# uw-x/AcousticSwarms-Speech

Hardware: AMD Instinct MI355X
Metric: TDoA candidates/sec (shift+normalise+spot forward+energies) (higher is better)
Workload: dtype f32 via f16x3 split-operand MFMA (fp32 accumulate); 1 GPU; configs[2] scene: 5-speaker reverberant mixture (image sources), 7 mics, T=48000 samples (BASELINE's '3 s @ 16 kHz' sample count; the reference pipeline and this scene generator run at 48 kHz, where it is a 1 s clip -- the reference-native 3 s is extras.T144000), fine-stage (Strict=1) candidate batch of one mixture, FULL spot net 47.27 M params, seeded random weights; internal_batch=256, parallelism=candidate-shard x1

## Files before the change

### acousticswarms-speech_amd/csrc/asw_common.cpp

```cpp
#include "asw_common.h"

#include <cmath>
#include <cstdlib>

namespace asw {
char* err_buf() {
  static thread_local char buf[512] = {0};
  return buf;
}
int set_error(int code, const char* fmt, ...) {
  va_list ap;
  va_start(ap, fmt);
  vsnprintf(err_buf(), 512, fmt, ap);
  va_end(ap);
  return code;
}
int SmemAttr::ensure(const void* kern, size_t want) {
  int dev = 0;
  ASW_HIP(hipGetDevice(&dev));
  if (dev < 0 || dev >= kMaxDev) return set_error(ASW_ERR_ARG, "device ordinal %d out of range", dev);
  if (bytes[dev] >= want) return ASW_OK;
  ASW_HIP(hipFuncSetAttribute(kern, hipFuncAttributeMaxDynamicSharedMemorySize, (int)want));
  bytes[dev] = want;
  return ASW_OK;
}
}

extern "C" const char* asw_last_error(void) { return asw::err_buf(); }
extern "C" int asw_abi_version(void) { return 3; }

extern "C" int asw_split_weights_f16(const float* w, size_t n, uint16_t* hi, uint16_t* lo, int32_t* w_shift) {
  ASW_CHECK_ARG(w && hi && lo && w_shift, "split_weights: null pointer");
  float mx = 0.f;
  for (size_t i = 0; i < n; ++i) { const float a = w[i] < 0 ? -w[i] : w[i]; if (a > mx || a != a) mx = a; }
  ASW_CHECK_ARG(mx == mx && mx < 3.0e38f, "split_weights: non-finite weight");
  int shift = 0;
  if (mx > 0.f) {
    int e;
    (void)frexpf(mx, &e);
    shift = 11 - e;
    if (shift > 24) shift = 24;
    if (shift < -24) shift = -24;
  }
  const float sc = ldexpf(1.0f, shift);
  for (size_t i = 0; i < n; ++i) {
    float c = w[i] * sc;
    if (c > 65504.f) c = 65504.f;
    if (c < -65504.f) c = -65504.f;
    const _Float16 h = (_Float16)c;
    const _Float16 l = (_Float16)(c - (float)h);
    memcpy(hi + i, &h, 2);
    memcpy(lo + i, &l, 2);
  }
  *w_shift = shift;
  return ASW_OK;
}

extern "C" int asw_pack_fragments_f16(const float* Wt, int N, int K, uint16_t* hi, uint16_t* lo, int32_t* w_shift) {
  ASW_CHECK_ARG(Wt && hi && lo && w_shift, "pack_fragments: null pointer");
  ASW_CHECK_ARG(N > 0 && K > 0 && N % 32 == 0 && K % 16 == 0, "pack_fragments: N %% 32, K %% 16 required (N=%d K=%d)", N, K);
  const size_t n = (size_t)N * K;
  uint16_t* th = new uint16_t[2 * n];
  uint16_t* tl = th + n;
  int rc = asw_split_weights_f16(Wt, n, th, tl, w_shift);
  if (rc == ASW_OK) {
    const int NT = N / 32;
    for (int ks = 0; ks < K / 16; ++ks)
      for (int nt = 0; nt < NT; ++nt)
        for (int l = 0; l < 64; ++l) {
          const size_t src = (size_t)(nt * 32 + (l & 31)) * K + ks * 16 + 8 * (l >> 5);
          const size_t dst = (((size_t)ks * NT + nt) * 64 + l) * 8;
          memcpy(hi + dst, th + src, 16);
          memcpy(lo + dst, tl + src, 16);
        }
  }
  delete[] th;
  return rc;
}

extern "C" int asw_up_feed_kperm(int k) { return (k & ~12) | ((k & 4) << 1) | ((k & 8) >> 1); }

extern "C" int asw_pack_up_feed_f16(const float* Wt, int N, int K, uint16_t* hi, uint16_t* lo, int32_t* w_shift) {
  ASW_CHECK_ARG(Wt && N > 0 && K > 0 && K % 16 == 0, "pack_up_feed: K %% 16 required (N=%d K=%d)", N, K);
  float* wp = new float[(size_t)N * K];
  for (int n = 0; n < N; ++n)
    for (int k = 0; k < K; ++k) wp[(size_t)n * K + k] = Wt[(size_t)n * K + (k & ~15) + asw_up_feed_kperm(k & 15)];
  const int rc = asw_pack_fragments_f16(wp, N, K, hi, lo, w_shift);
  delete[] wp;
  return rc;
}

namespace asw {
bool residue_feed_on() {
  static const bool off = getenv("ASW_NO_RESIDUE_FEED") != nullptr;
  return !off;
}
}

extern "C" int asw_residue_schedule(int taps, int stride, int dil, int pad, int Cin, int BK, int BM, int m0, int has_skip,
                                    asw_residue_stage* out, int cap, int* n_stages, int* max_shift) {
  ASW_CHECK_ARG(n_stages != nullptr && cap >= 0 && (out != nullptr || cap == 0), "residue_schedule: null pointer");
  ASW_CHECK_ARG(taps > 0 && stride > 0 && dil > 0 && Cin > 0 && BK > 0 && BM > 0, "residue_schedule: bad dims");
  *n_stages = 0;
  if (max_shift) *max_shift = 0;
  if (!asw::residue_feed_applies(taps, stride, dil, Cin, BK, has_skip != 0)) return ASW_OK;
  const asw::ResidueFeed rf{taps, stride, Cin / BK};
  ASW_CHECK_ARG(rf.ntaps(0) <= ASW_RESIDUE_MAX_TAPS, "residue_schedule: %d taps on one image, at most %d", rf.ntaps(0),
                ASW_RESIDUE_MAX_TAPS);
  *n_stages = rf.stages();
  if (max_shift) *max_shift = rf.shifts(0);
  for (int s = 0; s < rf.stages() && s < cap; ++s) {
    asw_residue_stage& d = out[s];
    memset(&d, 0, sizeof d);
    d.residue = s / rf.cpb;
    d.chunk = s - d.residue * rf.cpb;
    d.rows = BM + rf.shifts(d.residue);
    d.first_row = m0 * stride - pad + d.residue;
    d.ntaps = rf.ntaps(d.residue);
    for (int q = 0; q < d.ntaps; ++q) {
      d.tap[q] = rf.tap(d.residue, q);
      d.shift[q] = q;
      d.kstep[q] = rf.kstep(d.tap[q], d.chunk, BK / 16);
    }
  }
  return ASW_OK;
}

#include <map>
#include <mutex>
#include <vector>
namespace asw {
namespace {
struct Rec { std::string name; double work, bytes; hipEvent_t e0, e1; };
std::mutex g_mu;
bool g_on = false;
bool g_detail = false;
std::vector<Rec> g_recs;
std::vector<hipEvent_t> g_pool;
hipEvent_t take_event() {
  if (!g_pool.empty()) { hipEvent_t e = g_pool.back(); g_pool.pop_back(); return e; }
  hipEvent_t e = nullptr;
  (void)hipEventCreate(&e);
  return e;
}
}

std::string prof_name(const char* base, int bm, int bn, int bk, bool ln, bool stats) {
  char b[96];
  snprintf(b, sizeof b, "%s<%d,%d,%d,%s>", base, bm, bn, bk, ln ? "ln" : stats ? "stats" : "plain");
  return b;
}
bool prof_detail() { return g_detail; }
ProfScope::ProfScope(hipStream_t s, const std::string& name, double work, double bytes) : slot(-1), stream(s) {
  if (!g_on) return;
  std::lock_guard<std::mutex> lk(g_mu);
  Rec r{name, work, bytes, take_event(), take_event()};
  (void)hipEventRecord(r.e0, s);
  g_recs.push_back(r);
  slot = (int)g_recs.size() - 1;
}
ProfScope::~ProfScope() {
  if (slot < 0) return;
  std::lock_guard<std::mutex> lk(g_mu);
  if (slot < (int)g_recs.size()) (void)hipEventRecord(g_recs[slot].e1, stream);
}
}

extern "C" int asw_profile_enable(int on) {
  std::lock_guard<std::mutex> lk(asw::g_mu);
  for (auto& r : asw::g_recs) { asw::g_pool.push_back(r.e0); asw::g_pool.push_back(r.e1); }
  asw::g_recs.clear();
  asw::g_on = on != 0;
  asw::g_detail = on == 2;
  return ASW_OK;
}

extern "C" int asw_profile_report(char* buf, size_t cap) {
  if (!buf || cap < 64) return asw::set_error(ASW_ERR_ARG, "profile_report: buffer too small");
  std::lock_guard<std::mutex> lk(asw::g_mu);
  struct Agg { long n = 0; double ms = 0, work = 0, bytes = 0; };
  std::map<std::string, Agg> agg;
  for (auto& r : asw::g_recs) {
    if (hipEventSynchronize(r.e1) != hipSuccess) continue;
    float ms = 0.f;
    if (hipEventElapsedTime(&ms, r.e0, r.e1) != hipSuccess) continue;
    Agg& a = agg[r.name];
    a.n += 1; a.ms += ms; a.work += r.work; a.bytes += r.bytes;
  }
  size_t off = 0;
  off += snprintf(buf + off, cap - off, "{");
  bool first = true;
  for (auto& kv : agg) {
    if (off + 256 >= cap) break;
    off += snprintf(buf + off, cap - off, "%s\"%s\":{\"launches\":%ld,\"ms\":%.6f,\"work\":%.6e,\"bytes\":%.6e}", first ? "" : ",",
                    kv.first.c_str(), kv.second.n, kv.second.ms, kv.second.work, kv.second.bytes);
    first = false;
  }
  snprintf(buf + off, cap - off, "}");
  return ASW_OK;
}
```

### acousticswarms-speech_amd/csrc/asw_common.h

```cpp
#pragma once
#include <hip/hip_runtime.h>

#include <cstdarg>
#include <cstdio>
#include <cstring>

#include "../../include/asw_hip.h"

namespace asw {

char* err_buf();
int set_error(int code, const char* fmt, ...);

#define ASW_CHECK_ARG(cond, ...)                                   \
  do {                                                             \
    if (!(cond)) return ::asw::set_error(ASW_ERR_ARG, __VA_ARGS__); \
  } while (0)

#define ASW_HIP(call)                                                                 \
  do {                                                                                \
    hipError_t _e = (call);                                                           \
    if (_e != hipSuccess)                                                             \
      return ::asw::set_error(ASW_ERR_HIP, "%s failed: %s (%s:%d)", #call,            \
                              hipGetErrorString(_e), __FILE__, __LINE__);             \
  } while (0)

#define ASW_LAUNCH_CHECK()                                                            \
  do {                                                                                \
    hipError_t _e = hipGetLastError();                                                \
    if (_e != hipSuccess)                                                             \
      return ::asw::set_error(ASW_ERR_HIP, "kernel launch failed: %s (%s:%d)",        \
                              hipGetErrorString(_e), __FILE__, __LINE__);             \
  } while (0)

static inline hipStream_t as_stream(void* s) { return reinterpret_cast<hipStream_t>(s); }

struct SmemAttr {
  static constexpr int kMaxDev = 64;
  size_t bytes[kMaxDev] = {};
  int ensure(const void* kern, size_t want);
};
static inline int cdiv(long a, long b) { return (int)((a + b - 1) / b); }

#ifdef __HIPCC__
#define ASW_HOST_DEVICE __host__ __device__
#else
#define ASW_HOST_DEVICE
#endif
struct ResidueFeed {
  int taps, stride, cpb;
  ASW_HOST_DEVICE int stages() const { return stride * cpb; }
  ASW_HOST_DEVICE int shifts(int r) const { return (taps - 1 - r) / stride; }
  ASW_HOST_DEVICE int ntaps(int r) const { return shifts(r) + 1; }
  ASW_HOST_DEVICE int tap(int r, int q) const { return r + q * stride; }
  ASW_HOST_DEVICE int kstep(int tap, int c, int KS) const { return (tap * cpb + c) * KS; }
};
inline bool residue_feed_applies(int taps, int stride, int dil, int Cin, int BK, bool skip) {
  return dil == 1 && stride >= 2 && taps > stride && BK > 0 && BK % 16 == 0 && Cin > 0 && Cin % BK == 0 && !skip;
}
bool residue_feed_on();
inline bool pipe_offsets_ok(const asw_convgemm_args& a) {
  return (int64_t)a.stride * a.a_row_stride < (1 << 20) && (int64_t)a.pad * a.a_row_stride < (1 << 20) &&
         (int64_t)a.taps * a.dil * a.a_row_stride < (1 << 20);
}
inline bool residue_feed_ok(const asw_convgemm_args& a, int BK) {
  return residue_feed_on() && residue_feed_applies(a.taps, a.stride, a.dil, a.Cin, BK, a.A2 != nullptr) &&
         (a.taps - 1) / a.stride <= ASW_RESIDUE_MAX_SHIFT;
}

#ifdef __HIPCC__
__device__ __forceinline__ float gn_glu_value(float a, float g, float m0, float r0, float m1, float r1, float ga, float ba,
                                              float gg, float bg) {
  const float av = __fmaf_rn(__fmul_rn(__fsub_rn(a, m0), r0), ga, ba);
  const float gv = __fmaf_rn(__fmul_rn(__fsub_rn(g, m1), r1), gg, bg);
  const float e = __builtin_amdgcn_exp2f(__fmul_rn(gv, -1.4426950408889634f));
  return __fmul_rn(av, __builtin_amdgcn_rcpf(__fadd_rn(1.0f, e)));
}
#endif

}

#include <string>
namespace asw {
std::string prof_name(const char* base, int bm, int bn, int bk, bool ln, bool stats);
bool prof_detail();
struct ProfScope {
  ProfScope(hipStream_t s, const std::string& name, double work, double bytes = 0.0);
  ~ProfScope();
  int slot;
  hipStream_t stream;
};

struct ShapeTag {
  char s[64] = "";
  ShapeTag(const asw_convgemm_args& a, char key, int val, const char* feed = "") {
    if (prof_detail())
      snprintf(s, sizeof s, "[B%d M%d N%d K%d %c%d%s]", a.B, a.M_out, a.N, a.taps * a.Cin, key, val, feed);
  }
};

#ifdef __HIPCC__
template <auto K1, auto K3, typename... Args>
int launch_pair(int precision, dim3 grid, dim3 block, size_t lds, size_t lds_limit, std::string name, const char* detail,
                double flops, double bytes, hipStream_t s, const Args&... args) {
  const bool x1 = precision == 2;
  auto kern = x1 ? K1 : K3;
  static SmemAttr attr[2];
  if (int rc = attr[x1].ensure(reinterpret_cast<const void*>(kern), lds_limit)) return rc;
  if (prof_detail()) name += detail;
  ProfScope prof(s, name, flops, bytes);
  hipLaunchKernelGGL(kern, grid, block, lds, s, args...);
  ASW_LAUNCH_CHECK();
  return ASW_OK;
}
#endif
}
```

### acousticswarms-speech_amd/csrc/resstack.hip

```cpp
#include <type_traits>

#include "asw_common.h"
#include "f16x3_tile.h"

namespace {
using namespace asw_mfma;

constexpr int C = 64;
constexpr int MAXL = 3;
constexpr int NW = 4, TM = 2, QD = 4;
constexpr int NTHR = 64 * NW, SROWS = NTHR / 16;
constexpr int R0 = 32 * NW * TM;

struct LayerDev {
  const half8* Wh;
  const half8* Wl;
  const float* bias;
  const float* gamma;
  const float* beta;
  int dil, pad;
  int halo;
  int nfrag;
  float scale;
};

struct KArgs {
  const float* x;
  float* out;
  const float* glu_raw;
  const float* glu_mr;
  const float* glu_gamma;
  const float* glu_beta;
  float* glu_out;
  const half8* src_h;
  const half8* src_l;
  const half8* Pre_h;
  const half8* Pre_l;
  float pre_up, pre_down;
  int B, T, taps, ntile, BM, img_rows;
  float eps;
  LayerDev L[MAXL];
};

constexpr int UPN = 256;
struct UpArgs {
  const half8* Wh;
  const half8* Wl;
  const float* bias;
  const float* skip;
  float* out;
  float* stats;
  float scale;
};
struct KArgsUp : KArgs { UpArgs u; };

#ifdef ASW_PHASE_TIMING
__device__ unsigned long long g_rs_cycles[6] = {0, 0, 0, 0, 0, 0};
struct PhaseClock {
  unsigned long long t[2 * MAXL + 2];
  __device__ __forceinline__ void mark(int i) { t[i] = __builtin_readcyclecounter(); }
  __device__ __forceinline__ void mark_after(int i, float sink) {
    asm volatile("" ::"v"(sink));
    mark(i);
  }
  template <int NL>
  __device__ __forceinline__ void report() const {
    if (threadIdx.x != 0 || NL > 2) return;
    atomicAdd(&g_rs_cycles[0], t[1] - t[0]);
    atomicAdd(&g_rs_cycles[1], t[2] - t[1]);
    if (NL == 2) {
      atomicAdd(&g_rs_cycles[2], t[3] - t[2]);
      atomicAdd(&g_rs_cycles[3], t[4] - t[3]);
    }
    atomicAdd(&g_rs_cycles[4], t[2 * NL + 1] - t[2 * NL]);
    atomicAdd(&g_rs_cycles[5], 1ull);
  }
};
#else
struct PhaseClock {
  __device__ __forceinline__ void mark(int) {}
  __device__ __forceinline__ void mark_after(int, float) {}
  template <int NL>
  __device__ __forceinline__ void report() const {}
};
#endif

__device__ __forceinline__ __amdgpu_buffer_rsrc_t src_rsrc(const half8* base, long rows) {
  return __builtin_amdgcn_make_buffer_rsrc(const_cast<half8*>(base), 0, (int)(rows * 16), 0x00020000);
}
__device__ __forceinline__ half8 src_load(__amdgpu_buffer_rsrc_t r, int row) {
  return __builtin_bit_cast(half8, __builtin_amdgcn_raw_buffer_load_b128(r, row >= 0 ? row * 16 : (int)0x80000000, 0, 0));
}

template <bool POLY, int PH>
struct RowMap {
  static constexpr int BMJ = R0 / PH;
  static_assert(BMJ % 32 == 0, "a row fragment must stay inside one phase");
  int T, taps, dil0, pad0, jb, pb, m0, BM, n_img, halo0;

  __device__ __forceinline__ RowMap(int tile, const KArgs& p) : T(p.T), taps(p.taps), dil0(p.L[0].dil), pad0(p.L[0].pad) {
    const int n_pb = POLY ? (dil0 + PH - 1) / PH : 1;
    jb = POLY ? tile / n_pb : 0;
    pb = POLY ? tile - jb * n_pb : 0;
    m0 = tile * p.BM;
    BM = p.BM;
    n_img = POLY ? PH * rj() : R0 + 2 * pad0;
    halo0 = p.L[0].halo;
  }
  __device__ __forceinline__ int rj() const { return BMJ + taps - 1; }

  __device__ __forceinline__ ImgSrc staged_from(int irow) const {
    int g;
    bool ok = irow < n_img;
    if (!POLY) {
      g = m0 - halo0 - pad0 + irow;
    } else {
      const int ph = pb * PH + irow / rj();
      const int jj = jb * BMJ + irow % rj() - (taps - 1) / 2;
      g = dil0 * jj + ph;
      ok = ok && ph < dil0 && jj >= 0;
    }
    return {g, ok && g >= 0 && g < T};
  }
  __device__ __forceinline__ bool delivers(int g) const { return g >= m0 && g < m0 + BM; }

  __device__ __forceinline__ int image_row(int frow) const { return POLY ? (frow / BMJ) * rj() + frow % BMJ : frow; }
  __device__ __forceinline__ int tap_rows(const LayerDev& Ld) const { return POLY ? 1 : Ld.dil; }
  __device__ __forceinline__ int centre_rows(const LayerDev& Ld, bool first) const { return POLY ? (taps - 1) / 2 : first ? pad0 : Ld.pad; }

  __device__ __forceinline__ bool handed_on(int frow, int halo) const {
    const int t = m0 - halo + frow;
    return t >= 0 && t < T;
  }
  __device__ __forceinline__ int phase(int frow) const { return pb * PH + frow / BMJ; }
  __device__ __forceinline__ int seq_row(int frow) const { return POLY ? dil0 * (jb * BMJ + frow % BMJ) + phase(frow) : m0 + frow; }
  __device__ __forceinline__ ImgSrc delivered(int frow) const {
    const int t = seq_row(frow);
    return {t, (POLY ? phase(frow) < dil0 : frow < BM) && t < T};
  }
  __device__ __forceinline__ int row_step() const { return POLY ? dil0 : 1; }
  __device__ __forceinline__ int run_rows(int f0) const {
    if (!POLY) return min(BM, T - m0) - f0;
    const int t0 = seq_row(f0);
    return (phase(f0) < dil0 && t0 < T) ? (T - 1 - t0) / dil0 + 1 : 0;
  }
};

__device__ __forceinline__ int frag_row(int wid, int i, int lane) { return (wid * TM + i) * 32 + (lane & 31); }

template <typename F>
__device__ __forceinline__ void for_each_fragment(int nf, const F& f) {
  static_assert(TM == 2, "one line per fragment");
  if (0 < nf) f(0);
  if (1 < nf) f(1);
}

template <typename F>
__device__ __forceinline__ void for_each_group(int h, const F& f) {
#pragma unroll
  for (int cb = 0; cb < 2; ++cb)
#pragma unroll
    for (int q = 0; q < 4; ++q) f(cb, q, cb * 32 + q * 8 + h * 4);
}
__device__ __forceinline__ float4 group4(const floatx16& a, int q) { return make_float4(a[q * 4 + 0], a[q * 4 + 1], a[q * 4 + 2], a[q * 4 + 3]); }

template <int NL>
__device__ __forceinline__ void load_layer_vectors(const KArgs& p, float* tab, int tid) {
  for (int i = tid; i < NL * 3 * 16; i += NTHR) {
    const int li = i / 48, w = (i - li * 48) / 16, c4 = i & 15;
    const float* src = w == 0 ? p.L[li].bias : w == 1 ? p.L[li].gamma : p.L[li].beta;
    reinterpret_cast<float4*>(tab)[i] = *reinterpret_cast<const float4*>(src + c4 * 4);
  }
}

template <bool GLU, int NTERM, typename Map>
__device__ __forceinline__ void stage_rows(const KArgs& p, const Map& map, int b, char* img, int tid) {
  const int T = map.T;
  const __amdgpu_buffer_rsrc_t rX = GLU ? act_rsrc(p.glu_raw + (long)b * T * 2 * C, (long)T * 2 * C)
                                        : act_rsrc(p.x + (long)b * T * C, (long)T * C);
  const int srow = tid >> 4, sc4 = tid & 15;
  const int R_img = map.n_img;
  GluCoef gc;
  if (GLU) {
    gc.stats(p.glu_mr, b);
    gc.affine(p.glu_gamma, p.glu_beta, C, sc4 * 4);
  }
  constexpr int SU = GLU ? 9 : 18;
  for (int r0 = 0; r0 < R_img; r0 += SROWS * SU) {
    float4 buf[SU];
    float4 gate[GLU ? SU : 1];
    bool okr[GLU ? SU : 1];
#pragma unroll
    for (int u = 0; u < SU; ++u) {
      const ImgSrc f = map.staged_from(r0 + u * SROWS + srow);
      if (GLU) {
        buf[u] = act_load4(rX, (long)f.g * 2 * C + sc4 * 4, f.ok);
        gate[u] = act_load4(rX, (long)f.g * 2 * C + C + sc4 * 4, f.ok);
        okr[u] = f.ok;
        __builtin_amdgcn_sched_barrier(0);
      } else {
        buf[u] = act_load4(rX, (long)f.g * C + sc4 * 4, f.ok);
      }
    }
    if (GLU) {
#pragma unroll
      for (int u = 0; u < SU; ++u) {
        const float4 o = gn_glu4(buf[u], gate[u], gc, okr[u]);
        buf[u] = o;
        if (p.glu_out && okr[u]) {
          const int g = map.staged_from(r0 + u * SROWS + srow).g;
          if (map.delivers(g)) *reinterpret_cast<float4*>(p.glu_out + ((long)b * T + g) * C + sc4 * 4) = o;
        }
      }
    }
#pragma unroll
    for (int u = 0; u < SU; ++u) {
      const int row = r0 + u * SROWS + srow;
      if (row < R_img) {
        half4 hi, lo;
        split4t<NTERM>(buf[u], hi, lo);
        *reinterpret_cast<half4*>(img + row * RS + IMG_HI + sc4 * 8) = hi;
        *reinterpret_cast<half4*>(img + row * RS + IMG_LO + sc4 * 8) = lo;
      }
    }
  }
}

template <int NL, typename Map>
__device__ __forceinline__ void source_layer0(const KArgs& p, const Map& map, int b, float* tab, int tid, floatx16 (&acc)[TM][2]) {
  const LayerDev& Ld = p.L[0];
  const int T = map.T, lane = tid & 63, wid = tid >> 6, h = lane >> 5;
  const __amdgpu_buffer_rsrc_t rH = src_rsrc(p.src_h + (long)b * T, T), rL = src_rsrc(p.src_l + (long)b * T, T);
  const int g0 = map.staged_from(frag_row(wid, 0, lane)).g;
  half8 xh[4][TM], xl[4][TM], rh[TM], rl[TM];
#pragma unroll
  for (int ks = 0; ks < 4; ++ks)
#pragma unroll
    for (int i = 0; i < TM; ++i) {
      xh[ks][i] = src_load(rH, g0 + i * 32 + 2 * ks + h);
      xl[ks][i] = src_load(rL, g0 + i * 32 + 2 * ks + h);
    }
#pragma unroll
  for (int i = 0; i < TM; ++i) {
    rh[i] = src_load(rH, g0 + i * 32 + map.centre_rows(Ld, true));
    rl[i] = src_load(rL, g0 + i * 32 + map.centre_rows(Ld, true));
  }
  half8 wh[2][2], wl[2][2];
  auto wload = [&](auto kgc, int slot) {
    constexpr int kg = decltype(kgc)::value;
#pragma unroll
    for (int cb = 0; cb < 2; ++cb) {
      if constexpr (kg < 4) frag_load<3>(Ld.Wh, Ld.Wl, (long)kg * 2 + cb, lane, wh[slot][cb], wl[slot][cb]);
      else frag_load<3>(p.Pre_h, p.Pre_l, (long)cb, lane, wh[slot][cb], wl[slot][cb]);
    }
  };
  wload(std::integral_constant<int, 0>{}, 0);
  wload(std::integral_constant<int, 1>{}, 1);
  load_layer_vectors<NL>(p, tab, tid);
  __syncthreads();
  auto kstep = [&](auto ksc) {
    constexpr int ks = decltype(ksc)::value;
#pragma unroll
    for (int i = 0; i < TM; ++i)
#pragma unroll
      for (int cb = 0; cb < 2; ++cb) mma3<3, true>(acc[i][cb], xh[ks][i], xl[ks][i], wh[ks & 1][cb], wl[ks & 1][cb]);
    if constexpr (ks + 2 <= 4) wload(std::integral_constant<int, ks + 2>{}, ks & 1);
    __builtin_amdgcn_sched_barrier(0);
  };
  kstep(std::integral_constant<int, 0>{});
  kstep(std::integral_constant<int, 1>{});
  kstep(std::integral_constant<int, 2>{});
  kstep(std::integral_constant<int, 3>{});
#pragma unroll
  for (int i = 0; i < TM; ++i) {
    for_each_group(h, [&](int cb, int q, int c0) __attribute__((always_inline)) {
      const float4 bi = *reinterpret_cast<const float4*>(tab + c0);
      const float bv[4] = {bi.x, bi.y, bi.z, bi.w};
#pragma unroll
      for (int j = 0; j < 4; ++j)
        acc[i][cb][q * 4 + j] = fmaxf(acc[i][cb][q * 4 + j] * Ld.scale + bv[j], 0.f) * p.pre_up;
    });
#pragma unroll
    for (int cb = 0; cb < 2; ++cb) mma3<3, true>(acc[i][cb], rh[i], rl[i], wh[0][cb], wl[0][cb]);
  }
}

template <int NTERM, typename Map>
__device__ __forceinline__ void conv_layer(const KArgs& p, const LayerDev& Ld, const Map& map, const char* img, int nf, int lane,
                                           int wid, floatx16 (&acc)[TM][2]) {
  const int taps = map.taps, h = lane >> 5;
  const int tapstep = map.tap_rows(Ld) * RS;
  auto run = [&](auto nfc) {
    constexpr int NF = decltype(nfc)::value;
    int xb[NF];
    floatx16 a[NF][2];
#pragma unroll
    for (int i = 0; i < NF; ++i) {
      xb[i] = (map.image_row((wid * TM + i) * 32) + (lane & 31)) * RS + h * 16;
      a[i][0] = acc[i][0];
      a[i][1] = acc[i][1];
    }
    kloop<NF, 2, QD, NTERM>(
        a, taps, [&](int tap, int i) __attribute__((always_inline)) { return img + xb[i] + tap * tapstep; }, Ld.Wh, Ld.Wl,
        [](int kg, int cb) __attribute__((always_inline)) { return (long)kg * 2 + cb; }, lane);
#pragma unroll
    for (int i = 0; i < NF; ++i) { acc[i][0] = a[i][0]; acc[i][1] = a[i][1]; }
  };
  if (nf >= TM) run(std::integral_constant<int, TM>{});
  else if (nf == 1) run(std::integral_constant<int, 1>{});
}

template <bool IN_ACC, bool FUSED_VAR, typename Map>
__device__ __forceinline__ void finish_rows(const KArgs& p, const LayerDev& Ld, const Map& map, const char* img, const float* tb,
                                            bool first, int nf, int lane, int wid, floatx16 (&acc)[TM][2]) {
  const int h = lane >> 5;
  const int cpad = map.centre_rows(Ld, first);
  for_each_fragment(nf, [&](int i) __attribute__((always_inline)) {
    const char* rrow = img + (map.image_row(frag_row(wid, i, lane)) + cpad) * RS;
    float s = 0.f;
    for_each_group(h, [&](int cb, int q, int c0) __attribute__((always_inline)) {
      const float4 bi = *reinterpret_cast<const float4*>(tb + c0);
      const half4 rh = *reinterpret_cast<const half4*>(rrow + IMG_HI + c0 * 2);
      const half4 rl = *reinterpret_cast<const half4*>(rrow + IMG_LO + c0 * 2);
      const float bv[4] = {bi.x, bi.y, bi.z, bi.w};
#pragma unroll
      for (int j = 0; j < 4; ++j) {
        float v;
        if constexpr (IN_ACC) {
          v = acc[i][cb][q * 4 + j] * p.pre_down;
        } else {
          v = fmaxf(acc[i][cb][q * 4 + j] * Ld.scale + bv[j], 0.f);
          v += (float)rh[j] + (float)rl[j];
        }
        acc[i][cb][q * 4 + j] = v;
        s += v;
      }
    });
    s += __shfl_xor(s, 32, 64);
    const float mean = s * (1.0f / C);
    float d = 0.f;
#pragma unroll
    for (int cb = 0; cb < 2; ++cb)
#pragma unroll
      for (int r = 0; r < 16; ++r) {
        const float cx = acc[i][cb][r] - mean;
        if (FUSED_VAR && cb * 16 + r < 26) {
          d = __builtin_fmaf(cx, cx, d);
        } else {
#pragma clang fp contract(off)
          d += cx * cx;
        }
      }
    d += __shfl_xor(d, 32, 64);
    const float rstd = 1.0f / sqrtf(d * (1.0f / C) + p.eps);
    for_each_group(h, [&](int cb, int q, int c0) __attribute__((always_inline)) {
      const float4 g4 = *reinterpret_cast<const float4*>(tb + 64 + c0);
      const float4 b4 = *reinterpret_cast<const float4*>(tb + 128 + c0);
      const float gv[4] = {g4.x, g4.y, g4.z, g4.w}, be[4] = {b4.x, b4.y, b4.z, b4.w};
#pragma unroll
      for (int j = 0; j < 4; ++j) acc[i][cb][q * 4 + j] = (acc[i][cb][q * 4 + j] - mean) * rstd * gv[j] + be[j];
    });
  });
}

template <int NTERM, typename Map>
__device__ __forceinline__ void hand_over(const LayerDev& Ld, const Map& map, char* img, int nf, int lane, int wid,
                                          const floatx16 (&acc)[TM][2]) {
  for_each_fragment(nf, [&](int i) __attribute__((always_inline)) {
    const int frow = frag_row(wid, i, lane);
    const bool inside = map.handed_on(frow, Ld.halo);
    char* wrow = img + frow * RS;
    for_each_group(lane >> 5, [&](int cb, int q, int c0) __attribute__((always_inline)) {
      float4 v = group4(acc[i][cb], q);
      if (!inside) v = make_float4(0.f, 0.f, 0.f, 0.f);
      half4 hi, lo;
      split4t<NTERM>(v, hi, lo);
      *reinterpret_cast<half4*>(wrow + IMG_HI + c0 * 2) = hi;
      *reinterpret_cast<half4*>(wrow + IMG_LO + c0 * 2) = lo;
    });
  });
}

template <int NTERM, typename Map>
__device__ __forceinline__ void up_feed(const KArgs& p, const UpArgs& u, const LayerDev& Ld, const Map& map, int b, int tile,
                                        char* smem, int tid, const floatx16 (&acc)[TM][2]) {
  const int T = map.T, lane = tid & 63, wid = tid >> 6, h = lane >> 5;
  const __amdgpu_buffer_rsrc_t rS = act_rsrc(u.skip + (long)b * T * C, (long)T * C);
  const int tstep = map.row_step();
  const int widu = __builtin_amdgcn_readfirstlane(wid);
  half8 xh[TM][4], xl[TM][4];
  int t0[TM], nv[TM];
#pragma unroll
  for (int i = 0; i < TM; ++i) {
    const int f0 = (widu * TM + i) * 32;
    t0[i] = map.seq_row(f0);
    const int lim = map.run_rows(f0);
    nv[i] = i < Ld.nfrag - widu * TM ? min(max(lim, 0), 32) : 0;
    const bool ok = (lane & 31) < nv[i];
    const long e0 = ((long)t0[i] + (long)(lane & 31) * tstep) * C + h * 4;
    float4 sk[8];
#pragma unroll
    for (int c8 = 0; c8 < 8; ++c8) sk[c8] = act_load4(rS, e0 + c8 * 8, ok);
    for_each_group(h, [&](int cb, int q, int) __attribute__((always_inline)) {
      const float4 s4 = sk[cb * 4 + q];
      const float4 v = make_float4(acc[i][cb][q * 4 + 0] + s4.x, acc[i][cb][q * 4 + 1] + s4.y,
                                   acc[i][cb][q * 4 + 2] + s4.z, acc[i][cb][q * 4 + 3] + s4.w);
      half4 hi, lo;
      split4t<NTERM>(v, hi, lo);
#pragma unroll
      for (int j = 0; j < 4; ++j) {
        xh[i][cb * 2 + (q >> 1)][(q & 1) * 4 + j] = hi[j];
        xl[i][cb * 2 + (q >> 1)][(q & 1) * 4 + j] = lo[j];
      }
    });
  }
  float st0 = 0.f, sq0 = 0.f, st1 = 0.f, sq1 = 0.f;
  __amdgpu_buffer_rsrc_t rO[TM];
#pragma unroll
  for (int i = 0; i < TM; ++i)
    rO[i] = __builtin_amdgcn_make_buffer_rsrc(u.out + ((long)b * T + t0[i]) * UPN, 0,
                                              nv[i] > 0 ? ((nv[i] - 1) * tstep + 1) * UPN * 4 : 0, 0x00020000);
  const int voff = (4 * h * tstep * UPN + (lane & 31)) * 4;
  const int rstep = tstep * UPN * 4;
  half8 wh[2][2], wl[2][2];
  auto wload = [&](int ks, int nb2, int slot) __attribute__((always_inline)) {
#pragma unroll
    for (int e = 0; e < 2; ++e) frag_load<NTERM>(u.Wh, u.Wl, (long)ks * (UPN / 32) + nb2 * 2 + e, lane, wh[slot][e], wl[slot][e]);
  };
  wload(0, 0, 0);
#pragma unroll 1
  for (int nb2 = 0; nb2 < UPN / 64; ++nb2) {
    floatx16 y[TM][2];
#pragma unroll
    for (int i = 0; i < TM; ++i)
#pragma unroll
      for (int e = 0; e < 2; ++e)
#pragma unroll
        for (int r = 0; r < 16; ++r) y[i][e][r] = 0.f;
    const float bv[2] = {u.bias[nb2 * 64 + (lane & 31)], u.bias[nb2 * 64 + 32 + (lane & 31)]};
#pragma unroll
    for (int ks = 0; ks < 4; ++ks) {
      if (ks < 3) wload(ks + 1, nb2, (ks + 1) & 1);
      else wload(0, nb2 + 1 < UPN / 64 ? nb2 + 1 : nb2, 0);
#pragma unroll
      for (int i = 0; i < TM; ++i)
#pragma unroll
        for (int e = 0; e < 2; ++e) mma3<NTERM, false>(y[i][e], xh[i][ks], xl[i][ks], wh[ks & 1][e], wl[ks & 1][e]);
    }
    float s1 = 0.f, s2 = 0.f;
#pragma unroll
    for (int i = 0; i < TM; ++i) {
      const bool whole = nv[i] == 32;
#pragma unroll
      for (int e = 0; e < 2; ++e)
#pragma unroll
        for (int r = 0; r < 16; ++r) {
          const float v = y[i][e][r] * u.scale + bv[e];
          __builtin_amdgcn_raw_buffer_store_b32(__builtin_bit_cast(int, v), rO[i],
                                                voff + ((r & 3) + 8 * (r >> 2)) * rstep + (nb2 * 64 + e * 32) * 4, 0, 0);
          const float m = (whole || acc_row(r, h) < nv[i]) ? v : 0.f;
          s1 += m;
          s2 += m * m;
        }
    }
    if (nb2 & 1) { st1 += s1; sq1 += s2; } else { st0 += s1; sq0 += s2; }
  }
  st0 = wave_sum(st0); sq0 = wave_sum(sq0); st1 = wave_sum(st1); sq1 = wave_sum(sq1);
  __syncthreads();
  float* red = reinterpret_cast<float*>(smem);
  if (lane == 0) { red[wid * 4 + 0] = st0; red[wid * 4 + 1] = sq0; red[wid * 4 + 2] = st1; red[wid * 4 + 3] = sq1; }
  __syncthreads();
  if (tid < 4) {
    float s = 0.f;
#pragma unroll
    for (int w = 0; w < NW; ++w) s += red[w * 4 + tid];
    u.stats[((long)b * p.ntile + tile) * 4 + tid] = s;
  }
}

template <typename Map>
__device__ __forceinline__ void store_rows(const KArgs& p, const Map& map, int b, int nf, int lane, int wid,
                                           const floatx16 (&acc)[TM][2]) {
  float* __restrict__ ob = p.out + (long)b * map.T * C;
  for_each_fragment(nf, [&](int i) __attribute__((always_inline)) {
    const ImgSrc o = map.delivered(frag_row(wid, i, lane));
    if (o.ok) {
      float* orow = ob + (long)o.g * C;
      for_each_group(lane >> 5, [&](int cb, int q, int c0) __attribute__((always_inline)) {
        *reinterpret_cast<float4*>(orow + c0) = group4(acc[i][cb], q);
      });
    }
  });
}

template <int NL, int PH, bool POLY, bool GLU, int NTERM, bool SRC = false, bool UP = false>
__global__ __launch_bounds__(NTHR) __attribute__((amdgpu_waves_per_eu(2)))
void resstack64_kernel(const std::conditional_t<UP, KArgsUp, KArgs> p) {
  static_assert(!UP || (!SRC && NTERM == 3), "UpFeed: f16x3, never source-fed");
  static_assert(!POLY || NL == 1, "polyphase row sets: single layers only");
  static_assert(!SRC || (!POLY && !GLU && NTERM == 3), "source-fed layer 0: contiguous tiles, f16x3");

  extern __shared__ __align__(16) char smem[];
  char* img = smem;
  float* tab = reinterpret_cast<float*>(smem + (size_t)p.img_rows * RS);

  const int tid = threadIdx.x, lane = tid & 63, wid = tid >> 6;
  int idx;
  if (!xcd_tile_run(p.B * p.ntile, idx)) return;
  const int b = idx / p.ntile, tile = idx - b * p.ntile;
  const RowMap<POLY, PH> map(tile, p);

  PhaseClock clk;
  clk.mark(0);
  if constexpr (!SRC) {
    load_layer_vectors<NL>(p, tab, tid);
    stage_rows<GLU, NTERM>(p, map, b, img, tid);
    __syncthreads();
  }
  clk.mark(1);

  floatx16 acc[TM][2];
  auto layer = [&](auto lic) {
    constexpr int li = decltype(lic)::value;
    constexpr bool fed = SRC && li == 0;
    const LayerDev& Ld = p.L[li];
    const int nf = Ld.nfrag - wid * TM;
#pragma unroll
    for (int i = 0; i < TM; ++i)
#pragma unroll
      for (int cb = 0; cb < 2; ++cb)
#pragma unroll
        for (int r = 0; r < 16; ++r) acc[i][cb][r] = 0.f;
    if constexpr (fed) source_layer0<NL>(p, map, b, tab, tid, acc);
    else conv_layer<NTERM>(p, Ld, map, img, nf, lane, wid, acc);
    clk.mark_after(2 + 2 * li, acc[0][0][0]);
    finish_rows<fed, UP>(p, Ld, map, img, tab + li * 192, li == 0, nf, lane, wid, acc);
    if constexpr (li < NL - 1) {
      if constexpr (!fed) __syncthreads();
      hand_over<NTERM>(Ld, map, img, nf, lane, wid, acc);
      __syncthreads();
    } else if constexpr (UP) {
      up_feed<NTERM>(p, p.u, Ld, map, b, tile, smem, tid, acc);
    } else {
      store_rows(p, map, b, nf, lane, wid, acc);
    }
    clk.mark(3 + 2 * li);
  };
  layer(std::integral_constant<int, 0>{});
  if constexpr (NL > 1) layer(std::integral_constant<int, 1>{});
  if constexpr (NL > 2) layer(std::integral_constant<int, 2>{});
  clk.report<NL>();
}

template <bool GLU, bool SRC, bool UP>
double stack_bytes(const KArgs& k) {
  const double rows = (double)k.B * k.T;
  if (SRC) return rows * (32 + C * 4);
  if (UP) return rows * 4 * ((GLU ? 3 : 2) * C + UPN);
  return rows * C * 4 * (GLU ? 3 : 2);
}

template <int NL, int PH, bool POLY, bool GLU, bool SRC, bool UP>
int launch_stack(const KArgs& k, const UpArgs* up, int precision, size_t smem, double flops, hipStream_t s) {
  char nm[128], detail[48] = "";
  snprintf(nm, sizeof nm, "resstack64<%d,%dx%d%s%s%s%s>", NL, NW, TM, POLY ? (PH == 1 ? ",poly1" : PH == 2 ? ",poly2" : ",poly4") : "",
           GLU ? ",glu" : "", SRC ? ",src" : "", UP ? ",up" : "");
  if (asw::prof_detail()) snprintf(detail, sizeof detail, "[B%d M%d d%d]", k.B, k.T, k.L[0].dil);
  std::conditional_t<UP, KArgsUp, KArgs> ka;
  static_cast<KArgs&>(ka) = k;
  if constexpr (UP) {
    ka.u = *up;
    flops += 2.0 * k.B * (double)k.T * C * UPN;
  }
  return asw::launch_pair<resstack64_kernel<NL, PH, POLY, GLU, (SRC || UP) ? 3 : 1, SRC, UP>, resstack64_kernel<NL, PH, POLY, GLU, 3, SRC, UP>>(
      precision, dim3(xcd_grid_run(k.B * k.ntile)), dim3(NTHR), smem, 160 * 1024, nm, detail, flops, stack_bytes<GLU, SRC, UP>(k), s, ka);
}

template <int NL, int PH, bool POLY>
int launch_staged(const KArgs& k, const UpArgs* up, bool glu, int precision, size_t smem, double flops, hipStream_t s) {
  if constexpr (!POLY) {
    if (glu) return up ? launch_stack<NL, PH, POLY, true, false, true>(k, up, precision, smem, flops, s)
                       : launch_stack<NL, PH, POLY, true, false, false>(k, up, precision, smem, flops, s);
  }
  return up ? launch_stack<NL, PH, POLY, false, false, true>(k, up, precision, smem, flops, s)
            : launch_stack<NL, PH, POLY, false, false, false>(k, up, precision, smem, flops, s);
}

struct TilePlan { bool poly; int PH, BM, ntile; };
TilePlan plan_tiles(int T, int n_layers, int dil0, int halo0, bool glu) {
  const int rpp = T / dil0;
  if (n_layers == 1 && dil0 >= 7 && rpp >= 48 && !glu) {
    const int PH = rpp >= R0 - 32 ? 1 : rpp >= R0 / 2 - 32 ? 2 : 4;
    return {true, PH, R0, asw::cdiv(asw::cdiv(T, dil0), R0 / PH) * asw::cdiv(dil0, PH)};
  }
  const int BM = R0 - 2 * halo0;
  return {false, 1, BM, BM > 0 ? asw::cdiv(T, BM) : 0};
}

int dispatch(const asw_resstack_args& a, KArgs& k, const UpArgs* up, bool glu, double flops, hipStream_t s) {
  const int dil0 = k.L[0].dil;
  const TilePlan tp = plan_tiles(a.T, a.n_layers, dil0, k.L[0].halo, glu);
  k.BM = tp.BM;
  k.ntile = tp.ntile;
  if (tp.poly) {
    const int PH = tp.PH;
    const int BMJ = R0 / PH;
    k.L[0].nfrag = NW * TM;
    k.img_rows = PH * (BMJ + a.taps - 1);
    const size_t smem = (size_t)k.img_rows * RS + 3 * 64 * sizeof(float);
    switch (PH) {
      case 1: return launch_staged<1, 1, true>(k, up, false, a.precision, smem, flops, s);
      case 2: return launch_staged<1, 2, true>(k, up, false, a.precision, smem, flops, s);
      default: return launch_staged<1, 4, true>(k, up, false, a.precision, smem, flops, s);
    }
  }
  ASW_CHECK_ARG(k.BM >= R0 / 2, "resstack: the later layers' halo (%d rows per side) leaves %d of %d rows; fuse fewer layers",
                k.L[0].halo, k.BM, R0);
  int rows = 0;
  for (int i = 0; i < a.n_layers; ++i) {
    k.L[i].nfrag = asw::cdiv(k.BM + 2 * k.L[i].halo, 32);
    const int r = 32 * k.L[i].nfrag + 2 * k.L[i].pad;
    rows = r > rows ? r : rows;
  }
  k.img_rows = rows;
  const size_t smem = (size_t)rows * RS + (size_t)a.n_layers * 3 * 64 * sizeof(float);
  ASW_CHECK_ARG(smem <= 160 * 1024, "resstack: image of %d rows exceeds LDS (dilation %d x %d taps too wide for a contiguous tile)",
                rows, dil0, a.taps);
  if (k.src_h) {
    ASW_CHECK_ARG(k.L[0].nfrag == NW * TM, "resstack: source-fed layer 0 computes %d of %d fragments", k.L[0].nfrag, NW * TM);
    return launch_stack<2, 1, false, false, true, false>(k, nullptr, a.precision, smem, flops, s);
  }
  switch (a.n_layers) {
    case 1: return launch_staged<1, 1, false>(k, up, glu, a.precision, smem, flops, s);
    case 2: return launch_staged<2, 1, false>(k, up, glu, a.precision, smem, flops, s);
    default: return launch_staged<3, 1, false>(k, up, glu, a.precision, smem, flops, s);
  }
}

}

#ifdef ASW_PHASE_TIMING
extern "C" int asw_debug_resstack_cycles(unsigned long long* out6, int reset) {
  ASW_HIP(hipMemcpyFromSymbol(out6, HIP_SYMBOL(g_rs_cycles), 6 * sizeof(unsigned long long)));
  if (reset) {
    const unsigned long long z[6] = {0, 0, 0, 0, 0, 0};
    ASW_HIP(hipMemcpyToSymbol(HIP_SYMBOL(g_rs_cycles), z, sizeof z));
  }
  return ASW_OK;
}
#endif

extern "C" int asw_compose_source_weights(const float* wc, const float* wpre, const float* bpre, int M, int taps, float* comp,
                                          float* pre16) {
  ASW_CHECK_ARG(wc && wpre && bpre && comp && pre16, "compose_source_weights: null pointer");
  ASW_CHECK_ARG(M >= 1 && M <= 7 && taps >= 1 && taps <= 7, "compose_source_weights: M=%d taps=%d (at most 7 each)", M, taps);
  for (int i = 0; i < C * 16; ++i) pre16[i] = 0.f;
  for (int i = 0; i < C * 64; ++i) comp[i] = 0.f;
  for (int c = 0; c < C; ++c) {
    for (int m = 0; m < M; ++m) pre16[c * 16 + m] = wpre[c * M + m];
    pre16[c * 16 + 7] = bpre[c];
  }
  for (int n = 0; n < C; ++n)
    for (int k = 0; k < taps; ++k)
      for (int j = 0; j < 8; ++j) {
        double acc = 0.0;
        for (int c = 0; c < C; ++c) acc += (double)wc[((size_t)n * C + c) * taps + k] * (double)pre16[c * 16 + j];
        comp[n * 64 + k * 8 + j] = (float)acc;
      }
  return ASW_OK;
}

extern "C" int asw_resstack_tiles(int T, int taps, int n_layers, const int32_t* dil, int glu) {
  ASW_CHECK_ARG(T > 0 && taps >= 3 && taps % 2 == 1 && n_layers >= 1 && n_layers <= MAXL && dil, "resstack_tiles: bad argument");
  int halo0 = 0;
  for (int i = 1; i < n_layers; ++i) halo0 += dil[i] * (taps - 1) / 2;
  const TilePlan t = plan_tiles(T, n_layers, dil[0], halo0, glu != 0);
  ASW_CHECK_ARG(t.BM >= R0 / 2, "resstack_tiles: the later layers' halo (%d rows per side) is too wide", halo0);
  return t.ntile;
}

extern "C" int asw_resstack64_f16x3(const asw_resstack_args* args, void* stream) {
  ASW_CHECK_ARG(args != nullptr, "resstack: null args");
  const asw_resstack_args& a = *args;
  hipStream_t s = asw::as_stream(stream);
  ASW_CHECK_ARG(a.C == C, "resstack: C=%d (64 only)", a.C);
  ASW_CHECK_ARG(a.n_layers >= 1 && a.n_layers <= MAXL, "resstack: 1..%d layers", MAXL);
  ASW_CHECK_ARG(a.taps >= 3 && a.taps <= 15 && a.taps % 2 == 1, "resstack: taps=%d (odd, 3..15)", a.taps);
  ASW_CHECK_ARG(a.precision == 1 || a.precision == 2, "resstack: precision 1 (f16x3) or 2 (single-pass f16)");
  ASW_CHECK_ARG(a.B > 0 && a.B <= (1 << 20) && a.T > 0 && (int64_t)a.T * 2 * C < ((int64_t)1 << 29), "resstack: bad B / T");
  ASW_CHECK_ARG((a.out || a.up_hi) && (a.x || a.glu_raw || a.src_hi), "resstack: null tensor");
  const bool glu = a.glu_raw != nullptr;
  if (glu) ASW_CHECK_ARG(a.glu_mr && a.glu_gamma && a.glu_beta, "resstack: GroupNorm + GLU on load needs the statistics / affine arrays");
  KArgs k = {};
  k.x = a.x; k.out = a.out; k.glu_raw = a.glu_raw; k.glu_mr = a.glu_mr; k.glu_gamma = a.glu_gamma; k.glu_beta = a.glu_beta;
  k.glu_out = glu ? a.glu_out : nullptr;
  k.B = a.B; k.T = a.T; k.taps = a.taps; k.eps = a.ln_eps;
  int halo = 0;
  for (int i = a.n_layers - 1; i >= 0; --i) {
    const asw_reslayer_desc& d = a.layer[i];
    ASW_CHECK_ARG(d.Wf_hi && d.Wf_lo && d.bias && d.ln_gamma && d.ln_beta && d.dil >= 1, "resstack: layer %d incomplete", i);
    LayerDev& L = k.L[i];
    L.Wh = reinterpret_cast<const half8*>(d.Wf_hi); L.Wl = reinterpret_cast<const half8*>(d.Wf_lo);
    L.bias = d.bias; L.gamma = d.ln_gamma; L.beta = d.ln_beta;
    L.dil = d.dil; L.pad = d.dil * (a.taps - 1) / 2; L.halo = halo;
    L.scale = ldexpf(1.0f, -d.w_shift);
    halo += L.pad;
  }
  double flops = 2.0 * a.B * (double)a.T * C * C * a.taps * a.n_layers;
  if (a.src_hi) {
    ASW_CHECK_ARG(a.src_lo && a.pre_hi && a.pre_lo && !a.x && !glu, "resstack: the source-fed form takes src_hi / src_lo / pre_hi / pre_lo and no x");
    ASW_CHECK_ARG(a.precision == 1 && a.n_layers == 2 && a.taps <= 7 && a.layer[0].dil == 1,
                  "resstack: source-fed layer 0 is f16x3, two layers, dilation 1, at most 7 taps");
    k.src_h = reinterpret_cast<const half8*>(a.src_hi); k.src_l = reinterpret_cast<const half8*>(a.src_lo);
    k.Pre_h = reinterpret_cast<const half8*>(a.pre_hi); k.Pre_l = reinterpret_cast<const half8*>(a.pre_lo);
    k.pre_up = ldexpf(1.0f, a.pre_shift); k.pre_down = ldexpf(1.0f, -a.pre_shift);
    flops = 2.0 * a.B * (double)a.T * C * (64 + 16 + C * a.taps);
  }
  UpArgs up = {};
  if (a.up_hi) {
    ASW_CHECK_ARG(a.up_lo && a.up_bias && a.up_skip && a.up_out && a.up_stats, "resstack: UpFeed needs up_lo / up_bias / up_skip / up_out / up_stats");
    ASW_CHECK_ARG(a.precision == 1 && !a.src_hi, "resstack: UpFeed is f16x3 and never source-fed");
    up.Wh = reinterpret_cast<const half8*>(a.up_hi); up.Wl = reinterpret_cast<const half8*>(a.up_lo);
    up.bias = a.up_bias; up.skip = a.up_skip; up.out = a.up_out; up.stats = a.up_stats;
    up.scale = ldexpf(1.0f, -a.up_shift);
  }
  return dispatch(a, k, a.up_hi ? &up : nullptr, glu, flops, s);
}
```

### acousticswarms-speech_amd/native.py

```python
import ctypes
import glob
import os
import subprocess
import sys
from ctypes import (POINTER, Structure, c_char_p, c_double, c_float, c_int, c_int32, c_int64,
                    c_long, c_size_t, c_void_p)

_HERE = os.path.dirname(os.path.abspath(__file__))
LIB_PATH = os.environ.get("ASW_LIB_PATH") or os.path.join(_HERE, "libasw_hip.so")
CSRC = os.path.join(_HERE, "csrc")
SOURCES = ["asw_common.cpp", "convgemm.hip", "resconv.hip", "pipegemm.hip", "resstack.hip", "downconv.hip", "prep_kernels.hip",
           "misc_kernels.hip", "attention.hip", "srp_kernels.hip",
           "pruner_kernels.hip", "geometry_kernels.hip", "cluster_kernels.hip",
           "search_host.cpp", "sep_kernels.hip", "spot_model.hip", "sep_model.hip", "bss_kernels.hip", "eval_kernels.hip",
           "longform_kernels.hip", "stft_kernels.hip", "room_kernels.hip", "augment_kernels.hip"]
EXTRA_FLAGS = {"geometry_kernels.hip": ["-ffp-contract=off"], "cluster_kernels.hip": ["-ffp-contract=off"],
               "eval_kernels.hip": ["-ffp-contract=off"], "room_kernels.hip": ["-ffp-contract=off"]}
OPS_PATH = os.path.join(_HERE, "libasw_torch_ops.so")
OPS_SOURCE = "torch_ops.cpp"


def build(force: bool = False, verbose: bool = False) -> str:
    from concurrent.futures import ThreadPoolExecutor
    hdrs = glob.glob(os.path.join(CSRC, "*.h")) + [os.path.join(os.path.dirname(_HERE), "include", "asw_hip.h")]
    hdr_time = max(os.path.getmtime(h) for h in hdrs)
    objdir = os.path.join(_HERE, "build")
    os.makedirs(objdir, exist_ok=True)
    jobs, objs = [], []
    for src in SOURCES:
        sp = os.path.join(CSRC, src)
        op = os.path.join(objdir, os.path.splitext(src)[0] + ".o")
        objs.append(op)
        if force or not os.path.exists(op) or os.path.getmtime(op) < max(os.path.getmtime(sp), hdr_time):
            jobs.append(["hipcc", "-O3", "--offload-arch=gfx950", "-std=c++17", "-fPIC"] + EXTRA_FLAGS.get(src, [])
                        + ["-c", sp, "-o", op])
    if not jobs and os.path.exists(LIB_PATH) and all(os.path.getmtime(LIB_PATH) >= os.path.getmtime(o) for o in objs):
        return LIB_PATH

    def run(cmd):
        if verbose:
            print(" ".join(cmd), file=sys.stderr)
        subprocess.run(cmd, check=True)
    with ThreadPoolExecutor(max_workers=min(6, max(1, len(jobs)))) as ex:
        list(ex.map(run, jobs))
    run(["hipcc", "--offload-arch=gfx950", "-fPIC", "-shared", "-o", LIB_PATH] + objs)
    return LIB_PATH


def build_torch_ops(force: bool = False, verbose: bool = False) -> str:
    import torch
    src = os.path.join(CSRC, OPS_SOURCE)
    hdr = os.path.join(os.path.dirname(_HERE), "include", "asw_hip.h")
    if not force and os.path.exists(OPS_PATH) and os.path.getmtime(OPS_PATH) >= max(
            os.path.getmtime(src), os.path.getmtime(hdr), os.path.getmtime(LIB_PATH)):
        return OPS_PATH
    ti = os.path.dirname(torch.__file__)
    cmd = ["hipcc", "-O2", "-std=c++17", "-fPIC", "-shared", "-D__HIP_PLATFORM_AMD__=1", "-DUSE_ROCM=1",
           f"-D_GLIBCXX_USE_CXX11_ABI={int(torch._C._GLIBCXX_USE_CXX11_ABI)}", "-w",
           f"-I{ti}/include", f"-I{ti}/include/torch/csrc/api/include", "-I/opt/rocm/include", src, "-o", OPS_PATH,
           f"-L{_HERE}", "-lasw_hip", f"-L{ti}/lib", "-ltorch", "-ltorch_cpu", "-lc10", "-lc10_hip", "-ltorch_hip",
           "-Wl,-rpath,$ORIGIN", f"-Wl,-rpath,{ti}/lib"]
    if verbose:
        print(" ".join(cmd), file=sys.stderr)
    subprocess.run(cmd, check=True)
    return OPS_PATH


class SpotConfigC(Structure):
    _fields_ = [("n_mics", c_int32), ("kernel_size", c_int32), ("depth", c_int32),
                ("stride_list", c_int32 * 8), ("channels", c_int32), ("growth", c_int32),
                ("encoder_channels", c_int32), ("encoder_kernel_size", c_int32),
                ("encoder_stride", c_int32), ("residual_layers", c_int32),
                ("residual_dilation_factor", c_int32), ("num_head", c_int32), ("ffw_dim", c_int32),
                ("num_transformer_layers", c_int32)]

    @classmethod
    def from_config(cls, cfg):
        s = cls()
        s.n_mics, s.kernel_size, s.depth = cfg.n_mics, cfg.kernel_size, cfg.depth
        for i, v in enumerate(cfg.stride_list):
            s.stride_list[i] = v
        s.channels, s.growth = cfg.channels, int(cfg.growth)
        s.encoder_channels, s.encoder_kernel_size = cfg.encoder_channels, cfg.encoder_kernel_size
        s.encoder_stride, s.residual_layers = cfg.encoder_stride, cfg.residual_layers
        s.residual_dilation_factor, s.num_head = cfg.residual_dilation_factor, cfg.num_head
        s.ffw_dim, s.num_transformer_layers = cfg.ffw_dim, cfg.num_transformer_layers
        return s


class SepConfigC(Structure):
    _fields_ = [("n_mics", c_int32), ("max_speakers", c_int32), ("kernel_size", c_int32), ("depth", c_int32),
                ("stride_list", c_int32 * 8), ("channels", c_int32), ("growth", c_int32),
                ("encoder_channels", c_int32), ("encoder_kernel_size", c_int32), ("encoder_stride", c_int32),
                ("residual_layers", c_int32), ("residual_dilation_factor", c_int32), ("num_head", c_int32),
                ("ffw_dim", c_int32), ("bottleneck_layers", c_int32), ("bottleneck_ksize", c_int32)]

    @classmethod
    def from_config(cls, cfg):
        s = cls()
        s.n_mics, s.max_speakers, s.kernel_size, s.depth = cfg.n_mics, cfg.max_speakers, cfg.kernel_size, cfg.depth
        for i, v in enumerate(cfg.stride_list):
            s.stride_list[i] = v
        s.channels, s.growth = cfg.channels, int(cfg.growth)
        s.encoder_channels, s.encoder_kernel_size = cfg.encoder_channels, cfg.encoder_kernel_size
        s.encoder_stride, s.residual_layers = cfg.encoder_stride, cfg.residual_layers
        s.residual_dilation_factor, s.num_head = cfg.residual_dilation_factor, cfg.num_head
        s.ffw_dim, s.bottleneck_layers, s.bottleneck_ksize = cfg.ffw_dim, cfg.bottleneck_layers, cfg.bottleneck_ksize
        return s


class ConvGemmArgs(Structure):
    _fields_ = [("A", c_void_p), ("A2", c_void_p), ("Wt", c_void_p), ("bias", c_void_p),
                ("resid", c_void_p), ("mul", c_void_p), ("ln_gamma", c_void_p), ("ln_beta", c_void_p),
                ("out", c_void_p), ("stats", c_void_p),
                ("B", c_int32), ("M_out", c_int32), ("N", c_int32), ("Cin", c_int32), ("taps", c_int32),
                ("stride", c_int32), ("dil", c_int32), ("pad", c_int32), ("a_row_stride", c_int32),
                ("a_batch_stride", c_int64), ("a_len", c_int64), ("chan_mod", c_int32), ("relu", c_int32),
                ("ln_eps", c_float), ("precision", c_int32), ("w_shift", c_int32), ("Wt_hi", c_void_p),
                ("Wt_lo", c_void_p), ("Wf_hi", c_void_p), ("Wf_lo", c_void_p), ("stats_stride", c_int32),
                ("glu_raw", c_void_p), ("glu_mr", c_void_p), ("glu_gamma", c_void_p), ("glu_beta", c_void_p),
                ("glu_out", c_void_p)]


class MaskPathArgs(Structure):
    _fields_ = [("enc", ConvGemmArgs), ("ref", c_void_p), ("ref_batch_stride", c_int64), ("ref_len", c_int64),
                ("ref_hop", c_int32), ("byp_k", c_int32), ("byp_taps", c_int32), ("byp_shift", c_int32),
                ("byp_hi", c_void_p), ("byp_lo", c_void_p), ("byp_bias", c_void_p), ("dec_hi", c_void_p),
                ("dec_lo", c_void_p), ("dec_shift", c_int32), ("dec_taps", c_int32), ("taps", c_void_p)]


class ResLayerDesc(Structure):
    _fields_ = [("Wf_hi", c_void_p), ("Wf_lo", c_void_p), ("bias", c_void_p), ("ln_gamma", c_void_p),
                ("ln_beta", c_void_p), ("dil", c_int32), ("w_shift", c_int32)]


class ResStackArgs(Structure):
    _fields_ = [("x", c_void_p), ("out", c_void_p), ("B", c_int32), ("T", c_int32), ("C", c_int32), ("taps", c_int32),
                ("n_layers", c_int32), ("precision", c_int32), ("ln_eps", c_float), ("layer", ResLayerDesc * 3),
                ("glu_raw", c_void_p), ("glu_mr", c_void_p), ("glu_gamma", c_void_p), ("glu_beta", c_void_p),
                ("glu_out", c_void_p), ("src_hi", c_void_p), ("src_lo", c_void_p), ("pre_hi", c_void_p), ("pre_lo", c_void_p),
                ("pre_shift", c_int32), ("up_hi", c_void_p), ("up_lo", c_void_p), ("up_shift", c_int32), ("up_bias", c_void_p),
                ("up_skip", c_void_p), ("up_out", c_void_p), ("up_stats", c_void_p)]


RESIDUE_MAX_TAPS = 8


class ResidueStage(Structure):
    _fields_ = [("residue", c_int32), ("chunk", c_int32), ("rows", c_int32), ("first_row", c_int32), ("ntaps", c_int32),
                ("tap", c_int32 * RESIDUE_MAX_TAPS), ("shift", c_int32 * RESIDUE_MAX_TAPS),
                ("kstep", c_int32 * RESIDUE_MAX_TAPS)]


SIGNATURES = {
    "asw_last_error": (c_char_p, []),
    "asw_abi_version": (c_int, []),
    "asw_profile_enable": (c_int, [c_int]),
    "asw_profile_report": (c_int, [c_char_p, c_size_t]),
    "asw_spot_create": (c_int, [POINTER(SpotConfigC), POINTER(c_void_p)]),
    "asw_spot_destroy": (None, [c_void_p]),
    "asw_spot_set_param": (c_int, [c_void_p, c_char_p, c_void_p, c_size_t]),
    "asw_spot_finalize": (c_int, [c_void_p]),
    "asw_spot_set_batch": (c_int, [c_void_p, c_int]),
    "asw_spot_set_precision": (c_int, [c_void_p, c_int]),
    "asw_spot_set_lanes": (c_int, [c_void_p, c_int]),
    "asw_split_weights_f16": (c_int, [c_void_p, c_size_t, c_void_p, c_void_p, POINTER(c_int32)]),
    "asw_pack_fragments_f16": (c_int, [c_void_p, c_int, c_int, c_void_p, c_void_p, POINTER(c_int32)]),
    "asw_spot_shift_and_sep": (c_int, [c_void_p, c_void_p, c_int, c_int, c_void_p, c_int, c_int, c_int,
                                       c_void_p, c_void_p, c_int, c_void_p]),
    "asw_spot_shift_and_sep_multi": (c_int, [c_void_p, c_void_p, c_int, c_int, c_int, c_void_p, c_void_p, c_int, c_int, c_int,
                                             c_void_p, c_void_p, c_int, c_void_p]),
    "asw_spot_forward": (c_int, [c_void_p, c_void_p, c_int, c_int, c_int, POINTER(c_float), c_void_p, c_void_p]),
    "asw_spot_set_fused_mask": (c_int, [c_void_p, c_int]),
    "asw_spot_set_source_stack": (c_int, [c_void_p, c_int]),
    "asw_spot_set_up_fusion": (c_int, [c_void_p, c_int]),
    "asw_spot_get_tap": (c_int, [c_void_p, c_char_p, c_void_p, c_size_t, POINTER(c_size_t), c_void_p]),
    "asw_sep_create": (c_int, [POINTER(SepConfigC), POINTER(c_void_p)]),
    "asw_sep_destroy": (None, [c_void_p]),
    "asw_sep_set_param": (c_int, [c_void_p, c_char_p, c_void_p, c_size_t]),
    "asw_sep_finalize": (c_int, [c_void_p]),
    "asw_sep_set_precision": (c_int, [c_void_p, c_int]),
    "asw_sep_infer": (c_int, [c_void_p, c_void_p, c_int, c_int, c_void_p, c_int, c_void_p, c_void_p]),
    "asw_sep_infer_batch": (c_int, [c_void_p, c_void_p, c_int, c_int, c_int, c_void_p, c_void_p, c_void_p, c_void_p]),
    "asw_sep_forward": (c_int, [c_void_p, c_void_p, c_int, c_int, c_int, c_int, c_void_p, c_void_p]),
    "asw_sep_forward_counts": (c_int, [c_void_p, c_void_p, c_int, c_int, c_int, c_int, c_void_p, c_void_p, c_void_p]),
    "asw_sep_get_config": (c_int, [c_void_p, POINTER(SepConfigC)]),
    "asw_sep_get_tap": (c_int, [c_void_p, c_char_p, c_void_p, c_size_t, POINTER(c_size_t), c_void_p]),
    "asw_joint_shift_stats": (c_int, [c_void_p, c_int, c_int, c_void_p, c_int, c_void_p, c_void_p, c_void_p, c_void_p]),
    "asw_joint_shift_stats_scratch_doubles": (c_int, []),
    "asw_joint_shift_stats_groups": (c_int, [c_void_p, c_int, c_int, c_void_p, c_void_p, c_int, c_void_p, c_void_p, c_void_p,
                                             c_void_p, c_void_p]),
    "asw_add_layernorm2": (c_int, [c_void_p, c_void_p, c_float, c_void_p, c_void_p, c_int, c_int, c_float, c_int,
                                   c_void_p, c_void_p, c_void_p]),
    "asw_glu_rows": (c_int, [c_void_p, c_long, c_int, c_void_p, c_void_p]),
    "asw_dwconv_ln_swish": (c_int, [c_void_p, c_void_p, c_void_p, c_void_p, c_void_p, c_int, c_int, c_int, c_int,
                                    c_float, c_void_p, c_void_p]),
    "asw_relpos_attention": (c_int, [c_void_p, c_void_p, c_void_p, c_void_p, c_int, c_int, c_int, c_int, c_float,
                                     c_void_p, c_void_p]),
    "asw_inter_attention": (c_int, [c_void_p, c_int, c_int, c_int, c_int, c_int, c_void_p, c_void_p]),
    "asw_inter_attention_groups": (c_int, [c_void_p, c_void_p, c_int, c_int, c_int, c_int, c_void_p, c_void_p]),
    "asw_shift_stats": (c_int, [c_void_p, c_int, c_int, c_void_p, c_int, c_int, c_void_p, c_void_p, c_void_p]),
    "asw_shift_norm_preproc": (c_int, [c_void_p, c_int, c_int, c_int, c_void_p, c_int, c_int, c_void_p, c_void_p,
                                       c_void_p, c_void_p, c_int, c_void_p, c_void_p, c_long, c_void_p]),
    "asw_shift_stats_multi": (c_int, [c_void_p, c_int, c_int, c_void_p, c_void_p, c_int, c_int, c_void_p, c_void_p, c_void_p]),
    "asw_shift_norm_preproc_multi": (c_int, [c_void_p, c_int, c_int, c_int, c_void_p, c_void_p, c_int, c_int, c_void_p,
                                             c_void_p, c_void_p, c_void_p, c_int, c_void_p, c_void_p, c_long, c_void_p]),
    "asw_shift_norm_src_multi": (c_int, [c_void_p, c_int, c_int, c_int, c_void_p, c_void_p, c_int, c_int, c_void_p,
                                         c_void_p, c_void_p, c_void_p, c_void_p, c_long, c_void_p]),
    "asw_pad_preproc": (c_int, [c_void_p, c_int, c_int, c_int, c_int, c_void_p, c_void_p, c_int, c_void_p,
                                c_void_p, c_long, c_void_p]),
    "asw_convgemm_f32": (c_int, [POINTER(ConvGemmArgs), c_void_p]),
    "asw_mask_path_f16x3": (c_int, [POINTER(MaskPathArgs), c_void_p]),
    "asw_mask_path_f16x3_scaled": (c_int, [POINTER(MaskPathArgs), c_void_p]),
    "asw_resstack64_f16x3": (c_int, [POINTER(ResStackArgs), c_void_p]),
    "asw_resstack_tiles": (c_int, [c_int, c_int, c_int, POINTER(c_int32), c_int]),
    "asw_up_feed_kperm": (c_int, [c_int]),
    "asw_pack_up_feed_f16": (c_int, [c_void_p, c_int, c_int, c_void_p, c_void_p, POINTER(c_int32)]),
    "asw_compose_source_weights": (c_int, [c_void_p, c_void_p, c_void_p, c_int, c_int, c_void_p, c_void_p]),
    "asw_convgemm_stats_tiles": (c_int, [c_int, c_int]),
    "asw_f16x3_overflow_count": (c_int, [c_int, POINTER(c_int32)]),
    "asw_residue_schedule": (c_int, [c_int, c_int, c_int, c_int, c_int, c_int, c_int, c_int, c_int,
                                     POINTER(ResidueStage), c_int, POINTER(c_int), POINTER(c_int)]),
    "asw_gn_glu": (c_int, [c_void_p, c_void_p, c_int, c_void_p, c_void_p, c_int, c_int, c_int, c_float, c_void_p,
                           c_void_p]),
    "asw_gn_finalize": (c_int, [c_void_p, c_int, c_int, c_int, c_int, c_float, c_void_p, c_void_p]),
    "asw_attention": (c_int, [c_void_p, c_int, c_int, c_int, c_int, c_void_p, c_void_p]),
    "asw_attention_prec": (c_int, [c_void_p, c_int, c_int, c_int, c_int, c_int, c_void_p, c_void_p]),
    "asw_overlap_add_unnorm": (c_int, [c_void_p, c_int, c_int, c_int, c_int, c_int, c_int, c_int, c_int, c_float,
                                       c_void_p, c_void_p, c_void_p, c_void_p]),
    "asw_overlap_add_parts": (c_int, [c_void_p, c_int, c_int, c_int, c_int, c_int, c_int, c_int, c_int, c_int, c_float,
                                      c_void_p, c_void_p, c_void_p, c_void_p]),
    "asw_energies": (c_int, [c_void_p, c_int, c_int, c_int, c_void_p, c_void_p, c_void_p]),
    "asw_pair_sisdr": (c_int, [c_void_p, c_int, c_int, c_void_p, c_void_p]),
    "asw_center_rows": (c_int, [c_void_p, c_int, c_int, c_void_p]),
    "asw_segment_sisdr": (c_int, [c_void_p, c_int, c_int, c_void_p, c_void_p, c_int, c_void_p, c_void_p]),
    "asw_voiced_segments_workspace_bytes": (c_size_t, [c_int, c_int]),
    "asw_voiced_segments": (c_int, [c_void_p, c_int, c_int, c_double, c_double, c_void_p, c_int, c_void_p, c_void_p,
                                    c_void_p, c_size_t, c_void_p]),
    "asw_fine_clusters_workspace_bytes": (c_size_t, [c_void_p, c_int]),
    "asw_fine_clusters": (c_int, [c_void_p, c_int, c_int, c_void_p, c_int, c_void_p, c_void_p, c_void_p, c_double,
                                  c_double, c_void_p, c_size_t, c_void_p, c_void_p, c_void_p, c_void_p]),
    "asw_global_clusters_workspace_bytes": (c_size_t, [c_int]),
    "asw_global_clusters": (c_int, [c_void_p, c_void_p, c_void_p, c_void_p, c_int, c_int, c_double, c_double, c_double,
                                    c_double, c_double, c_void_p, c_size_t, c_void_p, c_void_p, c_void_p]),
    "asw_coarse_select_workspace_bytes": (c_size_t, [c_int, c_int]),
    "asw_coarse_select": (c_int, [c_void_p, c_void_p, c_void_p, c_int, c_double, c_int, c_double, c_int, c_void_p, c_size_t,
                                  c_void_p, c_void_p, c_void_p, c_void_p]),
    "asw_bss_eval_sdr_workspace_bytes": (c_size_t, [c_void_p, c_int, c_int, c_int, c_int]),
    "asw_bss_eval_sdr": (c_int, [c_void_p, c_void_p, c_void_p, c_int, c_int, c_int, c_int, c_void_p, c_void_p, c_void_p,
                                 c_size_t, c_void_p]),
    "asw_bss_eval_sources_workspace_bytes": (c_size_t, [c_void_p, c_int, c_int, c_int, c_int, c_int]),
    "asw_bss_eval_sources": (c_int, [c_void_p, c_void_p, c_void_p, c_int, c_int, c_int, c_int, c_int, c_void_p, c_void_p,
                                     c_void_p, c_void_p, c_void_p, c_size_t, c_void_p]),
    "asw_cross_sisdr_workspace_bytes": (c_size_t, [c_void_p, c_void_p, c_int, c_int]),
    "asw_cross_sisdr": (c_int, [c_void_p, c_void_p, c_void_p, c_void_p, c_int, c_int, c_void_p, c_void_p, c_void_p, c_size_t,
                                c_void_p]),
    "asw_add_layernorm": (c_int, [c_void_p, c_void_p, c_void_p, c_void_p, c_int, c_int, c_float, c_void_p, c_void_p]),
    "asw_search_area": (c_int, [c_void_p, c_int, c_void_p, c_int, c_void_p, c_void_p, c_void_p, c_double, c_double,
                                POINTER(c_int), POINTER(c_void_p), POINTER(c_void_p), POINTER(c_void_p),
                                POINTER(c_void_p)]),
    "asw_free": (None, [c_void_p]),
    "asw_cube_select": (c_int, [c_void_p, c_int, c_int, c_int, c_int, c_int, c_int, c_int, c_int, c_void_p, c_void_p,
                                c_void_p, c_int64, POINTER(c_int64)]),
    "asw_cube_select_planes": (c_int, [c_void_p, c_int, c_int, c_int, c_int, c_int, c_int, c_int, c_int, c_void_p, c_void_p,
                                c_void_p, c_int64, POINTER(c_int64)]),
    "asw_srp_frames": (c_int, [c_int, c_int, c_int]),
    "asw_srp_cross_spectra": (c_int, [c_void_p, c_int, c_int, c_int, c_int, c_int, c_int, c_int, c_int, c_int,
                                      c_float, c_void_p, c_void_p, c_void_p, c_int, c_void_p, c_void_p, c_void_p]),
    "asw_srp_map": (c_int, [c_void_p, c_int, c_int, c_int, c_void_p, c_int, c_int, c_void_p, c_void_p, c_void_p,
                            c_void_p, c_void_p, c_void_p]),
    "asw_pruner_covariance": (c_int, [c_void_p, c_int, c_int, c_int, c_int, c_int, c_int, c_int, c_int, c_int,
                                      c_void_p, c_void_p, c_void_p]),
    "asw_hermitian_eigh": (c_int, [c_void_p, c_int, c_int, c_void_p, c_void_p, c_void_p]),
    "asw_music_map": (c_int, [c_void_p, c_int, c_int, c_int, c_void_p, c_int, c_void_p, c_void_p, c_void_p, c_void_p,
                              c_void_p]),
    "asw_tops_map": (c_int, [c_void_p, c_void_p, c_int, c_int, c_int, c_int, c_void_p, c_int, c_double, c_void_p,
                             c_void_p, c_void_p, c_void_p]),
    "asw_geom_lookup_planes": (c_int, [c_void_p, c_int, c_void_p, c_int, c_void_p, c_int, c_void_p, c_int, c_double, c_double,
                                       c_void_p, c_void_p]),
    "asw_geom_voxel_map": (c_int, [c_void_p, c_int, c_void_p, c_int, c_void_p, c_int, c_void_p, c_int, c_void_p, c_void_p,
                                   c_double, c_double, c_double, c_void_p, c_void_p, c_void_p, c_void_p]),
    "asw_geom_label": (c_int, [c_void_p, c_void_p, c_int, c_int, c_int, c_int, c_void_p, c_void_p, c_void_p, POINTER(c_int),
                               c_void_p]),
    "asw_geom_workspace_bytes": (c_int64, [c_int]),
    "asw_geom_compact": (c_int, [c_void_p, c_void_p, c_void_p, c_int, c_void_p, c_int, c_void_p, c_int, c_void_p, c_int,
                                 c_void_p, c_double, c_void_p, c_int64, c_void_p, c_void_p, c_void_p, c_void_p, c_void_p,
                                 c_void_p, c_void_p, c_void_p, c_void_p, POINTER(c_int), c_void_p]),
    "asw_geom_lattice_workspace_bytes": (c_int64, [c_int, c_int]),
    "asw_geom_lattice": (c_int, [c_void_p, c_int, c_int, c_int, c_int, c_void_p, c_void_p, c_void_p, c_void_p, c_double,
                                 c_void_p, c_int64, c_void_p, c_void_p, c_void_p, c_void_p, POINTER(c_int), c_void_p]),
    "asw_lattice_nms_workspace_bytes": (c_int64, [c_int, c_int]),
    "asw_lattice_nms": (c_int, [c_void_p, c_int, c_int, c_void_p, c_int, c_void_p, c_int64, c_void_p, c_void_p, c_void_p]),
    "asw_frame_blocks": (c_int, [c_void_p, c_int, c_int, c_void_p, c_int, c_int, c_void_p, c_void_p]),
    "asw_stitch_blocks": (c_int, [c_void_p, c_int, c_void_p, c_void_p, c_void_p, c_int, c_int, c_int, c_int, c_void_p,
                                  c_void_p]),
    "asw_stft": (c_int, [c_void_p, c_int, c_int, c_void_p, c_void_p]),
    "asw_istft_workspace_bytes": (c_size_t, [c_int, c_int]),
    "asw_istft": (c_int, [c_void_p, c_int, c_int, c_int, c_void_p, c_void_p, c_size_t, c_void_p]),
    "asw_oracle_masks_workspace_bytes": (c_size_t, [c_void_p, c_void_p, c_int]),
    "asw_oracle_masks": (c_int, [c_void_p, c_void_p, c_void_p, c_void_p, c_int, c_int, c_int, c_double, c_double, c_void_p,
                                 c_void_p, c_size_t, c_void_p]),
    "asw_room_rir_workspace_bytes": (c_size_t, [c_int, c_int, c_int]),
    "asw_room_rir": (c_int, [c_void_p, c_void_p, c_void_p, c_void_p, c_void_p, c_void_p, c_int, c_int, c_double, c_int, c_void_p,
                             c_void_p, c_size_t, c_void_p]),
    "asw_room_convolve_workspace_bytes": (c_size_t, [c_void_p, c_int, c_int, c_int, c_int]),
    "asw_room_convolve": (c_int, [c_void_p, c_void_p, c_void_p, c_int, c_int, c_int, c_int, c_void_p, c_void_p, c_void_p,
                                  c_size_t, c_void_p]),
    "asw_colored_noise_workspace_bytes": (c_size_t, [c_int, c_int, c_int]),
    "asw_colored_noise": (c_int, [c_void_p, c_void_p, c_int, c_int, c_double, c_int, c_void_p, c_void_p, c_size_t, c_void_p]),
    "asw_train_batch_workspace_bytes": (c_size_t, [c_int, c_int, c_int]),
    "asw_train_batch": (c_int, [c_void_p, c_int, c_int, c_int, c_int, c_int, c_void_p, c_void_p, c_void_p, c_void_p, c_void_p,
                                c_void_p, c_void_p, c_void_p, c_int, c_void_p, c_size_t, c_void_p]),
    "asw_train_losses": (c_int, [c_void_p, c_void_p, c_int, c_int, c_void_p, c_void_p]),
}

_lib = None


def lib():
    global _lib
    if _lib is None:
        if not os.path.exists(LIB_PATH):
            raise RuntimeError(
                f"{LIB_PATH} is missing: run `python -c 'import __graft_entry__ as g; g.build()'` "
                "(hipcc --offload-arch=gfx950).  There is no CPU fallback for the hot path.")
        import torch
        L = ctypes.CDLL(LIB_PATH)
        for name, (res, args) in SIGNATURES.items():
            fn = getattr(L, name)
            fn.restype = res
            fn.argtypes = args
        _lib = L
    return _lib


_ops = None


def torch_ops():
    global _ops
    if _ops is None:
        lib()
        if not os.path.exists(OPS_PATH):
            raise RuntimeError(f"{OPS_PATH} is missing: run `python -c 'import __graft_entry__ as g; g.build()'`.  "
                               "The hot path is exposed only through these custom ops; there is no fallback.")
        import torch
        torch.ops.load_library(OPS_PATH)
        _ops = torch.ops.asw
    return _ops


def residue_schedule(taps, stride, Cin, BK=32, BM=256, m0=0, dil=1, pad=0, has_skip=False):
    n, mx = c_int(), c_int()
    L = lib()
    check(L.asw_residue_schedule(taps, stride, dil, pad, Cin, BK, BM, m0, int(has_skip), None, 0, ctypes.byref(n),
                                 ctypes.byref(mx)))
    if n.value == 0:
        return None
    buf = (ResidueStage * n.value)()
    check(L.asw_residue_schedule(taps, stride, dil, pad, Cin, BK, BM, m0, int(has_skip), buf, n.value, ctypes.byref(n),
                                 ctypes.byref(mx)))
    stages = [{"residue": d.residue, "chunk": d.chunk, "rows": d.rows, "first_row": d.first_row,
               "taps": [(d.tap[q], d.shift[q], d.kstep[q]) for q in range(d.ntaps)]} for d in buf]
    return stages, mx.value


def check(status: int):
    if status != 0:
        msg = lib().asw_last_error()
        raise RuntimeError(f"libasw_hip: status {status}: {msg.decode() if msg else ''}")


def ptr(t):
    return None if t is None else c_void_p(t.data_ptr())


def current_stream():
    import torch
    return c_void_p(torch.cuda.current_stream().cuda_stream)


def to_device(a, device):
    import torch
    src = torch.from_numpy(a)
    host = torch.empty(src.shape, dtype=src.dtype, pin_memory=True)
    host.copy_(src)
    return host.to(device, non_blocking=True)


def to_host(t):
    import torch
    if not t.is_cuda:
        return t.numpy()
    host = torch.empty(t.shape, dtype=t.dtype, pin_memory=True)
    host.copy_(t)
    return host.numpy()


def read_back(*tensors):
    import torch
    if not tensors:
        return []
    flat = [t.contiguous().reshape(-1).view(torch.uint8) for t in tensors]
    back = torch.cat(flat).cpu()
    out, pos = [], 0
    for t, f in zip(tensors, flat):
        piece = back[pos:pos + f.numel()].clone()
        out.append(piece.view(t.dtype).reshape(t.shape).numpy())
        pos += f.numel()
    return out
```

### acousticswarms-speech_amd/ops.py

```python
from ctypes import byref

import torch

from .native import ConvGemmArgs, MaskPathArgs, ResStackArgs, check, current_stream, lib, ptr


def _f32(t):
    assert t.is_cuda and t.dtype == torch.float32 and t.is_contiguous(), "need contiguous float32 CUDA tensor"
    return t


def pack_conv_weight(w: torch.Tensor) -> torch.Tensor:
    N, Cin, K = w.shape
    return w.permute(0, 2, 1).reshape(N, K * Cin).contiguous()


def convgemm(A, Wt, M_out, N, Cin, taps=1, stride=1, dil=1, pad=0, bias=None, relu=False, resid=None, mul=None,
             ln=None, stats_chan_mod=0, A2=None, B=None, a_row_stride=None, a_batch_stride=None, a_len=None,
             out=None, ln_eps=1e-5, precision="f32", use_fragments=True, glu=None, glu_out=None):
    _f32(A); _f32(Wt)
    if B is None:
        B = A.shape[0]
    a_row_stride = Cin if a_row_stride is None else a_row_stride
    if a_batch_stride is None:
        a_batch_stride = A[0].numel()
    if a_len is None:
        a_len = a_batch_stride
    if out is None:
        out = torch.empty((B, M_out, N), dtype=torch.float32, device=A.device)
    stats = None
    if stats_chan_mod:
        tiles = lib().asw_convgemm_stats_tiles(M_out, N)
        stats = torch.zeros((B, tiles, 4), dtype=torch.float32, device=A.device)
    a = ConvGemmArgs()
    a.A, a.A2, a.Wt = A.data_ptr(), (A2.data_ptr() if A2 is not None else None), Wt.data_ptr()
    a.bias = bias.data_ptr() if bias is not None else None
    a.resid = resid.data_ptr() if resid is not None else None
    a.mul = mul.data_ptr() if mul is not None else None
    a.ln_gamma = ln[0].data_ptr() if ln is not None else None
    a.ln_beta = ln[1].data_ptr() if ln is not None else None
    a.out = out.data_ptr()
    a.stats = stats.data_ptr() if stats is not None else None
    a.B, a.M_out, a.N, a.Cin, a.taps, a.stride, a.dil, a.pad = B, M_out, N, Cin, taps, stride, dil, pad
    a.a_row_stride, a.a_batch_stride, a.a_len = a_row_stride, a_batch_stride, a_len
    a.chan_mod, a.relu, a.ln_eps = stats_chan_mod, int(relu), ln_eps
    if glu is not None:
        a.glu_raw, a.glu_mr, a.glu_gamma, a.glu_beta = (_f32(t).data_ptr() for t in glu)
        if glu_out is not None:
            a.glu_out = _f32(glu_out).data_ptr()
    keep = None
    if precision in ("f16x3", "f16"):
        hi, lo, shift = split_weights_f16(Wt)
        keep = (hi, lo)
        a.precision, a.w_shift, a.Wt_hi, a.Wt_lo = (1 if precision == "f16x3" else 2), shift, hi.data_ptr(), lo.data_ptr()
        if use_fragments and N % 32 == 0 and (taps * Cin) % 16 == 0:
            fh, fl, sh2 = pack_fragments_f16(Wt, N, taps * Cin)
            assert sh2 == shift
            keep = keep + (fh, fl)
            a.Wf_hi, a.Wf_lo = fh.data_ptr(), fl.data_ptr()
    check(lib().asw_convgemm_f32(byref(a), current_stream()))
    torch.cuda.current_stream().synchronize() if keep is not None else None
    return out, stats


def _resstack_args(B, T, layers, taps, precision, eps, x=None, glu=None, glu_out=None, k0=None):
    a = ResStackArgs()
    a.x = _f32(x).data_ptr() if x is not None else None
    a.B, a.T, a.C, a.taps, a.n_layers = B, T, 64, taps, len(layers)
    a.precision, a.ln_eps = (1 if precision == "f16x3" else 2), eps
    keep = []
    for i, (Wt, bias, gamma, beta, dil) in enumerate(layers):
        fh, fl, sh = pack_fragments_f16(_f32(Wt), 64, k0 if (i == 0 and k0) else taps * 64)
        keep.append((fh, fl))
        d = a.layer[i]
        d.Wf_hi, d.Wf_lo, d.w_shift, d.dil = fh.data_ptr(), fl.data_ptr(), sh, dil
        d.bias, d.ln_gamma, d.ln_beta = _f32(bias).data_ptr(), _f32(gamma).data_ptr(), _f32(beta).data_ptr()
    if glu is not None:
        a.glu_raw, a.glu_mr, a.glu_gamma, a.glu_beta = (_f32(t).data_ptr() for t in glu)
        if glu_out is not None:
            a.glu_out = _f32(glu_out).data_ptr()
    return a, keep


def _resstack_launch(a):
    check(lib().asw_resstack64_f16x3(byref(a), current_stream()))
    torch.cuda.current_stream().synchronize()


def resstack(x, layers, taps=7, precision="f16x3", eps=1e-5, glu=None, out=None, glu_out=None):
    src = x if glu is None else glu[0]
    B, T = src.shape[0], src.shape[1]
    if out is None:
        out = torch.empty((B, T, 64), dtype=torch.float32, device=src.device)
    a, keep = _resstack_args(B, T, layers, taps, precision, eps, x=x, glu=glu, glu_out=glu_out)
    a.out = out.data_ptr()
    _resstack_launch(a)
    return out


def resstack_up(x, layers, up_wt, up_bias, skip, taps=7, eps=1e-5, glu=None):
    import ctypes
    src = x if glu is None else glu[0]
    B, T = src.shape[0], src.shape[1]
    dev = src.device
    a, keep = _resstack_args(B, T, layers, taps, "f16x3", eps, x=x, glu=glu)
    dils = (ctypes.c_int32 * 3)(*([l[4] for l in layers] + [1] * (3 - len(layers))))
    tiles = lib().asw_resstack_tiles(T, taps, len(layers), dils, int(glu is not None))
    check(min(tiles, 0))
    uh, ul, ush = pack_fragments_f16(up_wt, 256, 64, up_feed=True)
    raw = torch.full((B, T, 256), float("nan"), dtype=torch.float32, device=dev)
    stats = torch.full((B, tiles, 4), float("nan"), dtype=torch.float32, device=dev)
    a.up_hi, a.up_lo, a.up_shift = uh.data_ptr(), ul.data_ptr(), ush
    a.up_bias, a.up_skip, a.up_out, a.up_stats = _f32(up_bias).data_ptr(), _f32(skip).data_ptr(), raw.data_ptr(), stats.data_ptr()
    _resstack_launch(a)
    return raw, stats


def resstack_src(src_hi, src_lo, pre_w, pre_b, layers, taps=7, eps=1e-5, out=None):
    import ctypes
    import numpy as np
    B, T = src_hi.shape[0], src_hi.shape[1]
    dev = src_hi.device
    if out is None:
        out = torch.empty((B, T, 64), dtype=torch.float32, device=dev)
    M = pre_w.shape[1]
    wc = np.ascontiguousarray(layers[0][0].detach().cpu().numpy(), dtype=np.float32)
    wp = np.ascontiguousarray(pre_w.detach().cpu().numpy(), dtype=np.float32).reshape(64, M)
    bp = np.ascontiguousarray(pre_b.detach().cpu().numpy(), dtype=np.float32)
    comp, pre16 = np.empty((64, 64), dtype=np.float32), np.empty((64, 16), dtype=np.float32)
    check(lib().asw_compose_source_weights(ctypes.c_void_p(wc.ctypes.data), ctypes.c_void_p(wp.ctypes.data),
                                           ctypes.c_void_p(bp.ctypes.data), M, taps, ctypes.c_void_p(comp.ctypes.data),
                                           ctypes.c_void_p(pre16.ctypes.data)))
    dev_layers = [(torch.from_numpy(comp).to(dev) if i == 0 else pack_conv_weight(l[0]).to(dev),) + tuple(l[1:])
                  for i, l in enumerate(layers)]
    a, keep = _resstack_args(B, T, dev_layers, taps, "f16x3", eps, k0=64)
    a.out = out.data_ptr()
    ph, pl, psh = pack_fragments_f16(torch.from_numpy(pre16).to(dev), 64, 16)
    a.src_hi, a.src_lo, a.pre_hi, a.pre_lo, a.pre_shift = src_hi.data_ptr(), src_lo.data_ptr(), ph.data_ptr(), pl.data_ptr(), psh
    _resstack_launch(a)
    return out


def pack_fragments_f16(Wt, N, K, up_feed=False):
    import ctypes
    import numpy as np
    w = np.ascontiguousarray(Wt.detach().cpu().numpy(), dtype=np.float32).reshape(N, K)
    hi = np.empty(w.size, dtype=np.uint16)
    lo = np.empty(w.size, dtype=np.uint16)
    sh = ctypes.c_int32()
    pack = lib().asw_pack_up_feed_f16 if up_feed else lib().asw_pack_fragments_f16
    check(pack(ctypes.c_void_p(w.ctypes.data), N, K, ctypes.c_void_p(hi.ctypes.data),
               ctypes.c_void_p(lo.ctypes.data), byref(sh)))
    dev = Wt.device
    return (torch.from_numpy(hi.view(np.int16)).to(dev), torch.from_numpy(lo.view(np.int16)).to(dev), sh.value)


def split_weights_f16(Wt):
    import ctypes
    import numpy as np
    w = np.ascontiguousarray(Wt.detach().cpu().numpy(), dtype=np.float32)
    hi = np.empty(w.size, dtype=np.uint16)
    lo = np.empty(w.size, dtype=np.uint16)
    sh = ctypes.c_int32()
    check(lib().asw_split_weights_f16(ctypes.c_void_p(w.ctypes.data), w.size, ctypes.c_void_p(hi.ctypes.data),
                                      ctypes.c_void_p(lo.ctypes.data), byref(sh)))
    dev = Wt.device
    return (torch.from_numpy(hi.view(np.int16)).to(dev), torch.from_numpy(lo.view(np.int16)).to(dev), sh.value)


def gn_glu(raw, stats, gamma, beta, eps=1e-5):
    B, T, C2 = raw.shape
    C = C2 // 2
    out = torch.empty((B, T, C), dtype=torch.float32, device=raw.device)
    check(lib().asw_gn_glu(ptr(_f32(raw)), ptr(_f32(stats)), stats.shape[1], ptr(_f32(gamma)), ptr(_f32(beta)),
                           B, T, C, eps, ptr(out), current_stream()))
    return out


def gn_finalize(stats, T, C, eps=1e-5):
    B = stats.shape[0]
    mr = torch.empty((B, 4), dtype=torch.float32, device=stats.device)
    check(lib().asw_gn_finalize(ptr(_f32(stats)), stats.shape[1], B, T, C, eps, ptr(mr), current_stream()))
    return mr


def add_layernorm(x, resid, gamma, beta, eps=1e-5):
    rows, N = x.shape
    out = torch.empty_like(x)
    check(lib().asw_add_layernorm(ptr(_f32(x)), ptr(_f32(resid)), ptr(_f32(gamma)), ptr(_f32(beta)), rows, N, eps,
                                  ptr(out), current_stream()))
    return out


def attention(qkv, nhead, precision="f32"):
    B, L, d3 = qkv.shape
    d = d3 // 3
    ctx = torch.empty((B, L, d), dtype=torch.float32, device=qkv.device)
    check(lib().asw_attention_prec(ptr(_f32(qkv)), B, L, d, nhead, {"f32": 0, "f16x3": 1, "f16": 2}[precision], ptr(ctx),
                                   current_stream()))
    return ctx


def shift_stats(mix, offsets, circular=True):
    M, T = mix.shape
    N = offsets.shape[0]
    mean = torch.empty((N,), dtype=torch.float32, device=mix.device)
    std = torch.empty((N,), dtype=torch.float32, device=mix.device)
    check(lib().asw_shift_stats(ptr(_f32(mix)), M, T, ptr(offsets), N, int(circular), ptr(mean), ptr(std),
                                current_stream()))
    return mean, std


def shift_norm_preproc(mix, offsets, mean, std, w, b, T_pad, circular=True):
    M, T = mix.shape
    N = offsets.shape[0]
    C = w.shape[0]
    x0 = torch.empty((N, T_pad, C), dtype=torch.float32, device=mix.device)
    refn = torch.zeros((N, T_pad), dtype=torch.float32, device=mix.device)
    check(lib().asw_shift_norm_preproc(ptr(_f32(mix)), M, T, T_pad, ptr(offsets), N, int(circular), ptr(mean),
                                       ptr(std), ptr(_f32(w)), ptr(_f32(b)), C, ptr(x0), ptr(refn), T_pad,
                                       current_stream()))
    return x0, refn


def shift_norm_src(mix, offsets, mean, std, T_pad, circular=True):
    M, T = mix.shape
    N = offsets.shape[0]
    hi = torch.empty((N, T_pad, 8), dtype=torch.float16, device=mix.device)
    lo = torch.empty((N, T_pad, 8), dtype=torch.float16, device=mix.device)
    refn = torch.zeros((N, T_pad), dtype=torch.float32, device=mix.device)
    check(lib().asw_shift_norm_src_multi(ptr(_f32(mix)), M, T, T_pad, ptr(offsets), None, N, int(circular), ptr(mean),
                                         ptr(std), ptr(hi), ptr(lo), ptr(refn), T_pad, current_stream()))
    return hi, lo, refn


def overlap_add_unnorm(D, taps, hop, t, trim_left, trim_right, bias, mean=None, std=None):
    B, F, ldd = D.shape
    out = torch.empty((B, t), dtype=torch.float32, device=D.device)
    check(lib().asw_overlap_add_unnorm(ptr(_f32(D)), B, F, ldd, taps, hop, t, trim_left, trim_right, float(bias),
                                       ptr(mean), ptr(std), ptr(out), current_stream()))
    return out


def overlap_add_parts(Dp, taps, hop, t, trim_left, trim_right, bias, mean=None, std=None):
    nparts, B, F, ldd = Dp.shape
    out = torch.empty((B, t), dtype=torch.float32, device=Dp.device)
    check(lib().asw_overlap_add_parts(ptr(_f32(Dp)), nparts, B, F, ldd, taps, hop, t, trim_left, trim_right,
                                      float(bias), ptr(mean), ptr(std), ptr(out), current_stream()))
    return out


def mask_path(x, ref, ref_hop, enc_w, enc_b, byp_w, byp_b, dec_w, frames, stride, pad, precision="f16x3", scaled=False):
    B, Tp, C = x.shape
    E, _, EK = enc_w.shape
    dev = x.device
    Wt = pack_conv_weight(enc_w).to(dev)
    fh, fl, sh = pack_fragments_f16(Wt, E, EK * C)
    wb = torch.zeros((E, 48), dtype=torch.float32)
    wb[:, :byp_w.shape[-1]] = byp_w[:, 0].cpu()
    bh, bl, bsh = pack_fragments_f16(wb.to(dev), E, 48)
    wd = torch.zeros((64, E), dtype=torch.float32)
    wd[:dec_w.shape[-1]] = dec_w[:, 0].t().cpu()
    dh, dl, dsh = pack_fragments_f16(wd.to(dev), 64, E)
    parts = torch.zeros((E // 256, B, frames, 64), dtype=torch.float32, device=dev)
    m = MaskPathArgs()
    a = m.enc
    a.A, a.bias = _f32(x).data_ptr(), (_f32(enc_b).data_ptr() if enc_b is not None else None)
    a.B, a.M_out, a.N, a.Cin, a.taps, a.stride, a.dil, a.pad = B, frames, E, C, EK, stride, 1, pad
    a.a_row_stride, a.a_batch_stride, a.a_len = C, Tp * C, Tp * C
    a.precision, a.w_shift, a.Wf_hi, a.Wf_lo = {"f16x3": 1, "f16": 2}[precision], sh, fh.data_ptr(), fl.data_ptr()
    m.ref, m.ref_batch_stride, m.ref_len, m.ref_hop = _f32(ref).data_ptr(), ref.shape[1], ref.shape[1], ref_hop
    m.byp_k, m.byp_taps, m.byp_shift = 48, byp_w.shape[-1], bsh
    m.byp_hi, m.byp_lo = bh.data_ptr(), bl.data_ptr()
    m.byp_bias = _f32(byp_b).data_ptr() if byp_b is not None else None
    m.dec_hi, m.dec_lo, m.dec_shift, m.dec_taps = dh.data_ptr(), dl.data_ptr(), dsh, dec_w.shape[-1]
    m.taps = parts.data_ptr()
    check((lib().asw_mask_path_f16x3_scaled if scaled else lib().asw_mask_path_f16x3)(byref(m), current_stream()))
    torch.cuda.current_stream().synchronize()
    return parts


def energies(y, window=12000):
    B, T = y.shape
    out = torch.empty((B, 2), dtype=torch.float64, device=y.device)
    check(lib().asw_energies(ptr(_f32(y)), B, T, window, None, ptr(out), current_stream()))
    return out


def pair_sisdr(y):
    n, T = y.shape
    out = torch.empty((n, n), dtype=torch.float64, device=y.device)
    check(lib().asw_pair_sisdr(ptr(_f32(y)), n, T, ptr(out), current_stream()))
    return out


def srp_cross_spectra(mix, twiddle, pair_i, pair_j, nbins, window, step, n_windows, nfft, hop, tol=1e-8):
    M, T = mix.shape
    P = pair_i.shape[0]
    nb_pad = twiddle.shape[0] // 2
    assert twiddle.shape == (2 * nb_pad, nfft), "twiddle must be [2*nb_pad, nfft]"
    for t in (pair_i, pair_j):
        assert t.is_cuda and t.dtype == torch.int32 and t.is_contiguous() and t.numel() == P, "pair tables: int32 [P]"
    F = lib().asw_srp_frames(window, nfft, hop)
    xf = torch.empty((M, max(F, 1), 2 * nb_pad), dtype=torch.float32, device=mix.device)
    cc = torch.full((n_windows, nbins, P, 2), float("nan"), dtype=torch.float32, device=mix.device)
    check(lib().asw_srp_cross_spectra(ptr(_f32(mix)), M, T, window, step, n_windows, nfft, hop, nbins, nb_pad, tol,
                                      ptr(_f32(twiddle)), ptr(pair_i), ptr(pair_j), P, ptr(xf), ptr(cc),
                                      current_stream()))
    return cc


def srp_map(cc, tau, omega, pair_i, pair_j):
    n_windows, nbins, P, _ = cc.shape
    G, M = tau.shape
    for t, dt, n in ((tau, torch.float64, G * M), (omega, torch.float64, nbins), (pair_i, torch.int32, P),
                     (pair_j, torch.int32, P)):
        assert t.is_cuda and t.dtype == dt and t.is_contiguous() and t.numel() == n, "srp_map: operand dtype / size"
    part = torch.empty((8 * 8 * G,), dtype=torch.float32, device=cc.device)
    out = torch.empty((G,), dtype=torch.float32, device=cc.device)
    check(lib().asw_srp_map(ptr(_f32(cc)), n_windows, nbins, P, ptr(tau), G, M, ptr(omega), ptr(pair_i), ptr(pair_j),
                            ptr(part), ptr(out), current_stream()))
    return out


def joint_shift_stats(mix, offsets):
    M, T = mix.shape
    S = offsets.shape[0]
    scratch = torch.empty((lib().asw_joint_shift_stats_scratch_doubles(),), dtype=torch.float64, device=mix.device)
    mean = torch.empty((S,), dtype=torch.float32, device=mix.device)
    std = torch.empty((S,), dtype=torch.float32, device=mix.device)
    check(lib().asw_joint_shift_stats(ptr(_f32(mix)), M, T, ptr(offsets), S, ptr(scratch), ptr(mean), ptr(std),
                                      current_stream()))
    return mean, std


def _group_tables(counts):
    import ctypes
    bounds, items = [0], []
    for k, c in enumerate(counts):
        if int(c) > 0:
            bounds.append(bounds[-1] + int(c))
            items.append(k)
    return (ctypes.c_int32 * len(bounds))(*bounds), (ctypes.c_int32 * max(1, len(items)))(*items), len(items)


def joint_shift_stats_groups(mix_stack, offsets, counts):
    K, M, T = mix_stack.shape
    N = offsets.shape[0]
    assert len(counts) == K and sum(int(c) for c in counts) == N and all(int(c) >= 0 for c in counts)
    assert offsets.is_cuda and offsets.dtype == torch.int32 and offsets.is_contiguous() and offsets.shape[1] == M - 1
    bounds, items, G = _group_tables(counts)
    scratch = torch.empty((max(1, G) * lib().asw_joint_shift_stats_scratch_doubles(),), dtype=torch.float64,
                          device=mix_stack.device)
    mean = torch.empty((N,), dtype=torch.float32, device=mix_stack.device)
    std = torch.empty((N,), dtype=torch.float32, device=mix_stack.device)
    check(lib().asw_joint_shift_stats_groups(ptr(_f32(mix_stack)), M, T, ptr(offsets), bounds, G, items, ptr(scratch),
                                             ptr(mean), ptr(std), current_stream()))
    return mean, std


def add_layernorm2(x, y=None, alpha=1.0, gamma=None, beta=None, eps=1e-5, act=0, want_sum=False, want_ln=True):
    rows, N = x.shape
    s = torch.empty_like(x) if want_sum else None
    o = torch.empty_like(x) if want_ln else None
    check(lib().asw_add_layernorm2(ptr(_f32(x)), ptr(y), float(alpha), ptr(gamma), ptr(beta), rows, N, eps, act, ptr(s),
                                   ptr(o), current_stream()))
    return s, o


def glu_rows(raw):
    rows, C2 = raw.shape
    out = torch.empty((rows, C2 // 2), dtype=torch.float32, device=raw.device)
    check(lib().asw_glu_rows(ptr(_f32(raw)), rows, C2 // 2, ptr(out), current_stream()))
    return out


def dwconv_ln_swish(u, w, bias, gamma, beta, eps=1e-5):
    BS, L, d = u.shape
    K = w.shape[-1]
    wT = w.reshape(d, K).t().contiguous()
    out = torch.empty_like(u)
    check(lib().asw_dwconv_ln_swish(ptr(_f32(u)), ptr(_f32(wT)), ptr(_f32(bias)), ptr(_f32(gamma)), ptr(_f32(beta)),
                                    BS, L, d, K, eps, ptr(out), current_stream()))
    return out


def relpos_attention(qkv, P, bias_u, bias_v, nhead, scale):
    BS, L, d3 = qkv.shape
    d = d3 // 3
    ctx = torch.empty((BS, L, d), dtype=torch.float32, device=qkv.device)
    check(lib().asw_relpos_attention(ptr(_f32(qkv)), ptr(_f32(P)), ptr(_f32(bias_u)), ptr(_f32(bias_v)), BS, L, d, nhead,
                                     float(scale), ptr(ctx), current_stream()))
    return ctx


def inter_attention(qkv, nhead):
    NB, S, L, d3 = qkv.shape
    d = d3 // 3
    ctx = torch.empty((NB, S, L, d), dtype=torch.float32, device=qkv.device)
    check(lib().asw_inter_attention(ptr(_f32(qkv)), NB, S, L, d, nhead, ptr(ctx), current_stream()))
    return ctx


def inter_attention_groups(qkv, counts, nhead, out=None):
    N, L, d3 = qkv.shape
    d = d3 // 3
    assert sum(int(c) for c in counts) == N and all(int(c) >= 0 for c in counts)
    bounds, _items, G = _group_tables(counts)
    ctx = torch.empty((N, L, d), dtype=torch.float32, device=qkv.device) if out is None else out
    assert ctx.shape == (N, L, d)
    check(lib().asw_inter_attention_groups(ptr(_f32(qkv)), bounds, G, L, d, nhead, ptr(_f32(ctx)), current_stream()))
    return ctx


def _host_i32(values):
    import ctypes
    flat = [int(v) for v in values]
    return (ctypes.c_int32 * max(1, len(flat)))(*flat)


def frame_blocks(mix, starts, T, out=None):
    M, Ttot = mix.shape
    K = len(starts)
    blocks = torch.empty((K, M, int(T)), dtype=torch.float32, device=mix.device) if out is None else out
    assert blocks.shape == (K, M, int(T))
    check(lib().asw_frame_blocks(ptr(_f32(mix)), M, Ttot, _host_i32(starts), K, int(T), ptr(_f32(blocks)), current_stream()))
    return blocks


def stitch_blocks(rows, taper, starts, row_of, Ttot, out=None):
    N, T = rows.shape
    K = len(starts)
    S = len(row_of[0])
    assert len(row_of) == K and all(len(r) == S for r in row_of)
    assert taper.is_cuda and taper.dtype == torch.float64 and taper.is_contiguous() and taper.shape == (T,)
    res = torch.empty((S, int(Ttot)), dtype=torch.float32, device=rows.device) if out is None else out
    assert res.shape == (S, int(Ttot))
    check(lib().asw_stitch_blocks(ptr(_f32(rows)), N, ptr(taper), _host_i32(starts), _host_i32(v for r in row_of for v in r), K, S,
                                  T, int(Ttot), ptr(_f32(res)), current_stream()))
    return res


def _ws_f64(nbytes, device):
    return torch.empty(((int(nbytes) + 7) // 8,), dtype=torch.float64, device=device)


def stft(x, out=None):
    from .oracle_masks import NBINS, frame_count
    R, N = x.shape
    F = frame_count(N)
    z = torch.empty((R, NBINS, F), dtype=torch.complex128, device=x.device) if out is None else out
    assert z.shape == (R, NBINS, F) and z.dtype == torch.complex128 and z.is_cuda and z.is_contiguous()
    check(lib().asw_stft(ptr(_f32(x)), R, N, ptr(z), current_stream()))
    return z


def istft(z, N, out=None):
    R, _nb, F = z.shape
    assert z.is_cuda and z.dtype == torch.complex128 and z.is_contiguous() and _nb == 1025
    res = torch.empty((R, int(N)), dtype=torch.float64, device=z.device) if out is None else out
    assert res.shape == (R, int(N)) and res.dtype == torch.float64 and res.is_cuda and res.is_contiguous()
    nbytes = lib().asw_istft_workspace_bytes(R, F)
    if nbytes == 0:
        check(-1)
    ws = _ws_f64(nbytes, z.device)
    check(lib().asw_istft(ptr(z), R, F, int(N), ptr(res), ptr(ws), nbytes, current_stream()))
    return res


ORACLE_KINDS = {"irm": 0, "ibm": 1}


def oracle_masks(mix, ref, counts, lengths, kind, alpha=1.0, theta=0.5, out=None):
    K, T = mix.shape
    assert len(counts) == K and len(lengths) == K and ref.shape == (sum(int(c) for c in counts), T)
    res = torch.empty((ref.shape[0], T), dtype=torch.float64, device=mix.device) if out is None else out
    assert res.shape == (ref.shape[0], T) and res.dtype == torch.float64 and res.is_cuda and res.is_contiguous()
    c, n = _host_i32(counts), _host_i32(lengths)
    nbytes = lib().asw_oracle_masks_workspace_bytes(c, n, K)
    if nbytes == 0:
        check(-1)
    ws = _ws_f64(nbytes, mix.device)
    check(lib().asw_oracle_masks(ptr(_f32(mix)), ptr(_f32(ref)) if ref.shape[0] else None, c, n, K, T, ORACLE_KINDS[kind],
                                 float(alpha), float(theta), ptr(res) if ref.shape[0] else None, ptr(ws), nbytes,
                                 current_stream()))
    return res


def _host_f64(a, shape):
    import numpy as np
    a = np.ascontiguousarray(np.asarray(a, dtype=np.float64))
    assert a.shape == tuple(shape), f"shape {a.shape}, expected {tuple(shape)}"
    return a


def room_rir(rooms, absorption, max_orders, src, mics, counts, fs, length, device=None, out=None):
    K = len(counts)
    NS = sum(int(c) for c in counts)
    import numpy as np
    M = np.shape(mics)[1]
    rooms, absorption, src = _host_f64(rooms, (K, 3)), _host_f64(absorption, (K,)), _host_f64(src, (NS, 3))
    mics = _host_f64(mics, (K, M, 3))
    assert len(max_orders) == K
    if device is None:
        device = torch.device("cuda", torch.cuda.current_device()) if out is None else out.device
    res = torch.empty((NS, M, int(length)), dtype=torch.float64, device=device) if out is None else out
    assert res.shape == (NS, M, int(length)) and res.dtype == torch.float64 and res.is_cuda and res.is_contiguous()
    nbytes = lib().asw_room_rir_workspace_bytes(K, M, NS)
    if nbytes == 0:
        check(-1)
    with torch.cuda.device(res.device):
        ws = _ws_f64(nbytes, res.device)
        check(lib().asw_room_rir(rooms.ctypes.data, absorption.ctypes.data, _host_i32(max_orders), src.ctypes.data, mics.ctypes.data,
                                 _host_i32(counts), K, M, float(fs), int(length), ptr(res), ptr(ws), nbytes, current_stream()))
    return res


def room_convolve(dry, rir, counts, out=None):
    NS, T = dry.shape
    _ns, M, length = rir.shape
    K = len(counts)
    assert _ns == NS == sum(int(c) for c in counts)
    assert rir.is_cuda and rir.dtype == torch.float64 and rir.is_contiguous()
    premix, mix = (torch.empty((NS, M, T), dtype=torch.float64, device=dry.device),
                   torch.empty((K, M, T), dtype=torch.float64, device=dry.device)) if out is None else out
    for t, shape in ((premix, (NS, M, T)), (mix, (K, M, T))):
        assert t.shape == shape and t.dtype == torch.float64 and t.is_cuda and t.is_contiguous()
    c = _host_i32(counts)
    nbytes = lib().asw_room_convolve_workspace_bytes(c, K, M, length, T)
    if nbytes == 0:
        check(-1)
    ws = _ws_f64(nbytes, dry.device)
    check(lib().asw_room_convolve(ptr(_f32(dry)) if NS else None, ptr(rir) if NS else None, c, K, M, length, T,
                                  ptr(premix) if NS else None, ptr(mix), ptr(ws), nbytes, current_stream()))
    return premix, mix


def _host_i64(values):
    import ctypes
    flat = [((int(v) + 2 ** 63) % 2 ** 64) - 2 ** 63 for v in values]
    return (ctypes.c_int64 * max(1, len(flat)))(*flat)


def _host_f64_list(values):
    import ctypes
    flat = [float(v) for v in values]
    return (ctypes.c_double * max(1, len(flat)))(*flat)


def colored_noise(key, rows, T, exponent=1.0, max_rows_per_pass=0, device=None, out=None):
    ids = list(range(rows)) if isinstance(rows, int) else [int(r) for r in rows]
    keys = [int(key)] * len(ids) if isinstance(key, int) else [int(k) for k in key]
    assert len(keys) == len(ids)
    n = len(ids)
    if device is None:
        device = torch.device("cuda", torch.cuda.current_device()) if out is None else out.device
    res = torch.empty((n, int(T)), dtype=torch.float64, device=device) if out is None else out
    assert res.shape == (n, int(T)) and res.dtype == torch.float64 and res.is_cuda and res.is_contiguous()
    nbytes = lib().asw_colored_noise_workspace_bytes(n, int(T), int(max_rows_per_pass))
    if nbytes == 0:
        check(-1)
    with torch.cuda.device(res.device):
        ws = _ws_f64(nbytes, res.device)
        check(lib().asw_colored_noise(_host_i64(keys), _host_i32(ids), n, int(T), float(exponent), int(max_rows_per_pass), ptr(res),
                                      ptr(ws), nbytes, current_stream()))
    return res


def train_batch(mix, item_mix, shifts, counts, pink_level, white_level, white_key, pink=None, dtype=torch.float32, out=None):
    import numpy as np
    K, M, T = mix.shape
    sh = np.ascontiguousarray(np.asarray(shifts, dtype=np.int32))
    n_items = len(item_mix)
    assert sh.ndim == 3 and sh.shape[0] == n_items and sh.shape[2] == M, f"shifts {sh.shape}: expected [{n_items}][S_max][{M}]"
    S = sh.shape[1]
    assert len(counts) == len(pink_level) == len(white_level) == len(white_key) == n_items
    assert dtype in (torch.float32, torch.float64)
    if pink is not None:
        assert pink.shape == (n_items, S * M, T) and pink.dtype == torch.float64 and pink.is_contiguous() and pink.device == mix.device
    res = torch.empty((n_items, S * M, T), dtype=dtype, device=mix.device) if out is None else out
    assert res.shape == (n_items, S * M, T) and res.dtype == dtype and res.is_cuda and res.is_contiguous()
    nbytes = lib().asw_train_batch_workspace_bytes(n_items, S, M)
    if nbytes == 0:
        check(-1)
    with torch.cuda.device(mix.device):
        ws = _ws_f64(nbytes, mix.device)
        check(lib().asw_train_batch(ptr(_f32(mix)), K, M, T, n_items, S, _host_i32(item_mix), sh.ctypes.data, _host_i32(counts),
                                    _host_f64_list(pink_level), _host_f64_list(white_level), _host_i64(white_key), ptr(pink), ptr(res),
                                    int(dtype == torch.float64), ptr(ws), nbytes, current_stream()))
    return res


def train_losses(est, gt, out=None):
    N, T = est.shape
    assert gt.shape == est.shape and gt.device == est.device
    res = torch.empty((N, 4), dtype=torch.float64, device=est.device) if out is None else out
    assert res.shape == (N, 4) and res.dtype == torch.float64 and res.is_cuda and res.is_contiguous()
    with torch.cuda.device(est.device):
        check(lib().asw_train_losses(ptr(_f32(est)), ptr(_f32(gt)), N, T, ptr(res), current_stream()))
    return res


def f16x3_overflow_count(reset=True) -> int:
    import ctypes
    c = ctypes.c_int32()
    check(lib().asw_f16x3_overflow_count(int(reset), byref(c)))
    return int(c.value) & 0xFFFFFFFF
```

### include/asw_hip.h

```cpp
#ifndef ASW_HIP_H
#define ASW_HIP_H

#include <stddef.h>
#include <stdint.h>

#ifdef __cplusplus
extern "C" {
#endif

typedef enum asw_status {
  ASW_OK = 0,
  ASW_ERR_ARG = -1,
  ASW_ERR_HIP = -2,
  ASW_ERR_NOMEM = -3,
  ASW_ERR_STATE = -4
} asw_status;

const char* asw_last_error(void);
int asw_abi_version(void);

int asw_profile_enable(int on);
int asw_profile_report(char* buf, size_t cap);

typedef struct asw_spot_config {
  int32_t n_mics;
  int32_t kernel_size;
  int32_t depth;
  int32_t stride_list[8];
  int32_t channels;
  int32_t growth;
  int32_t encoder_channels;
  int32_t encoder_kernel_size;
  int32_t encoder_stride;
  int32_t residual_layers;
  int32_t residual_dilation_factor;
  int32_t num_head;
  int32_t ffw_dim;
  int32_t num_transformer_layers;
} asw_spot_config;

typedef struct asw_spot asw_spot;

int asw_spot_create(const asw_spot_config* cfg, asw_spot** out);
void asw_spot_destroy(asw_spot* m);

int asw_spot_set_param(asw_spot* m, const char* key, const float* host_data, size_t numel);
int asw_spot_finalize(asw_spot* m);

int asw_spot_set_batch(asw_spot* m, int batch);

int asw_spot_set_lanes(asw_spot* m, int lanes);

int asw_spot_set_precision(asw_spot* m, int precision);

int asw_spot_shift_and_sep(asw_spot* m, const float* mix, int M, int T,
                           const int32_t* offsets, int N, int strict, int circular,
                           float* out_wave, double* out_energy, int energy_window,
                           void* stream);

int asw_spot_shift_and_sep_multi(asw_spot* m, const float* mix, int K, int M, int T, const int32_t* offsets,
                                 const int32_t* mix_index, int N, int strict, int circular, float* out_wave,
                                 double* out_energy, int energy_window, void* stream);

int asw_spot_forward(asw_spot* m, const float* mix_norm, int B, int M, int t,
                     const float* window_embedding_host, float* out, void* stream);

int asw_spot_set_fused_mask(asw_spot* m, int on);

int asw_spot_set_source_stack(asw_spot* m, int on);

int asw_spot_set_up_fusion(asw_spot* m, int on);

int asw_spot_get_tap(asw_spot* m, const char* name, float* dst, size_t capacity, size_t* numel,
                     void* stream);

typedef struct asw_sep_config {
  int32_t n_mics;
  int32_t max_speakers;
  int32_t kernel_size;
  int32_t depth;
  int32_t stride_list[8];
  int32_t channels;
  int32_t growth;
  int32_t encoder_channels;
  int32_t encoder_kernel_size;
  int32_t encoder_stride;
  int32_t residual_layers;
  int32_t residual_dilation_factor;
  int32_t num_head;
  int32_t ffw_dim;
  int32_t bottleneck_layers;
  int32_t bottleneck_ksize;
} asw_sep_config;

typedef struct asw_sep asw_sep;

int asw_sep_create(const asw_sep_config* cfg, asw_sep** out);
void asw_sep_destroy(asw_sep* m);
int asw_sep_set_param(asw_sep* m, const char* key, const float* host_data, size_t numel);
int asw_sep_finalize(asw_sep* m);
int asw_sep_set_precision(asw_sep* m, int precision);

int asw_sep_infer(asw_sep* m, const float* mix, int M, int T, const int32_t* offsets, int S, float* out,
                  void* stream);

int asw_sep_infer_batch(asw_sep* m, const float* mix, int K, int M, int T, const int32_t* offsets,
                        const int32_t* counts, float* out, void* stream);

int asw_sep_forward(asw_sep* m, const float* mix_norm, int B, int S, int M, int t, float* out, void* stream);
int asw_sep_forward_counts(asw_sep* m, const float* mix_norm, int B, int S, int M, int t, const int32_t* counts,
                           float* out, void* stream);
int asw_sep_get_config(const asw_sep* m, asw_sep_config* out);

int asw_sep_get_tap(asw_sep* m, const char* name, float* dst, size_t capacity, size_t* numel, void* stream);

int asw_joint_shift_stats(const float* mix, int M, int T, const int32_t* offsets, int S, double* scratch,
                          float* mean, float* std, void* stream);
int asw_joint_shift_stats_scratch_doubles(void);
int asw_joint_shift_stats_groups(const float* mix, int M, int T, const int32_t* offsets, const int32_t* bounds, int G,
                                 const int32_t* item_of_group, double* scratch, float* mean, float* std, void* stream);

int asw_add_layernorm2(const float* x, const float* y, float alpha, const float* gamma, const float* beta,
                       int rows, int N, float eps, int act, float* sum_out, float* ln_out, void* stream);

int asw_glu_rows(const float* raw, long rows, int C, float* out, void* stream);

int asw_dwconv_ln_swish(const float* u, const float* wT, const float* bias, const float* gamma, const float* beta,
                        int BS, int L, int d, int K, float eps, float* out, void* stream);

int asw_relpos_attention(const float* qkv, const float* P, const float* bias_u, const float* bias_v, int BS, int L,
                         int d, int nhead, float scale, float* ctx, void* stream);

int asw_inter_attention(const float* qkv, int NB, int S, int L, int d, int nhead, float* ctx, void* stream);
int asw_inter_attention_groups(const float* qkv, const int32_t* bounds, int G, int L, int d, int nhead, float* ctx,
                               void* stream);


int asw_shift_stats(const float* mix, int M, int T, const int32_t* offsets, int N,
                    int circular, float* mean, float* std, void* stream);

int asw_shift_norm_preproc(const float* mix, int M, int T, int T_pad, const int32_t* offsets,
                           int N, int circular, const float* mean, const float* std,
                           const float* w, const float* b, int C, float* x0, float* refn,
                           long refn_stride, void* stream);

int asw_shift_stats_multi(const float* mix, int M, int T, const int32_t* offsets, const int32_t* mix_index, int N,
                          int circular, float* mean, float* std, void* stream);
int asw_shift_norm_preproc_multi(const float* mix, int M, int T, int T_pad, const int32_t* offsets,
                                 const int32_t* mix_index, int N, int circular, const float* mean, const float* std,
                                 const float* w, const float* b, int C, float* x0, float* refn, long refn_stride,
                                 void* stream);

int asw_shift_norm_src_multi(const float* mix, int M, int T, int T_pad, const int32_t* offsets,
                             const int32_t* mix_index, int N, int circular, const float* mean, const float* std,
                             void* src_hi, void* src_lo, float* refn, long refn_stride, void* stream);

int asw_pad_preproc(const float* x, int B, int M, int t, int T_pad, const float* w,
                    const float* b, int C, float* x0, float* refn, long refn_stride,
                    void* stream);

typedef struct asw_convgemm_args {
  const float* A;
  const float* A2;
  const float* Wt;
  const float* bias;
  const float* resid;
  const float* mul;
  const float* ln_gamma;
  const float* ln_beta;
  float* out;
  float* stats;
  int32_t B, M_out, N, Cin, taps, stride, dil, pad;
  int32_t a_row_stride;
  int64_t a_batch_stride;
  int64_t a_len;
  int32_t chan_mod;
  int32_t relu;
  float ln_eps;
  int32_t precision;
  int32_t w_shift;
  const void* Wt_hi;
  const void* Wt_lo;
  const void* Wf_hi;
  const void* Wf_lo;
  int32_t stats_stride;
  const float* glu_raw;
  const float* glu_mr;
  const float* glu_gamma;
  const float* glu_beta;
  float* glu_out;
} asw_convgemm_args;
int asw_pack_fragments_f16(const float* Wt, int N, int K, uint16_t* hi, uint16_t* lo, int32_t* w_shift);
int asw_convgemm_f32(const asw_convgemm_args* args, void* stream);
typedef struct asw_maskpath_args {
  asw_convgemm_args enc;
  const float* ref;
  int64_t ref_batch_stride;
  int64_t ref_len;
  int32_t ref_hop;
  int32_t byp_k;
  int32_t byp_taps;
  int32_t byp_shift;
  const void* byp_hi;
  const void* byp_lo;
  const float* byp_bias;
  const void* dec_hi;
  const void* dec_lo;
  int32_t dec_shift;
  int32_t dec_taps;
  float* taps;
} asw_maskpath_args;
int asw_mask_path_f16x3(const asw_maskpath_args* args, void* stream);
int asw_mask_path_f16x3_scaled(const asw_maskpath_args* args, void* stream);
typedef struct asw_reslayer_desc {
  const void* Wf_hi;
  const void* Wf_lo;
  const float* bias;
  const float* ln_gamma;
  const float* ln_beta;
  int32_t dil;
  int32_t w_shift;
} asw_reslayer_desc;
typedef struct asw_resstack_args {
  const float* x;
  float* out;
  int32_t B, T, C, taps, n_layers;
  int32_t precision;
  float ln_eps;
  asw_reslayer_desc layer[3];
  const float* glu_raw;
  const float* glu_mr;
  const float* glu_gamma;
  const float* glu_beta;
  float* glu_out;
  const void* src_hi;
  const void* src_lo;
  const void* pre_hi;
  const void* pre_lo;
  int32_t pre_shift;
  const void* up_hi;
  const void* up_lo;
  int32_t up_shift;
  const float* up_bias;
  const float* up_skip;
  float* up_out;
  float* up_stats;
} asw_resstack_args;
int asw_resstack64_f16x3(const asw_resstack_args* args, void* stream);
int asw_resstack_tiles(int T, int taps, int n_layers, const int32_t* dil, int glu);
int asw_up_feed_kperm(int k);
int asw_pack_up_feed_f16(const float* Wt, int N, int K, uint16_t* hi, uint16_t* lo, int32_t* w_shift);
int asw_compose_source_weights(const float* wc, const float* wpre, const float* bpre, int M, int taps, float* comp,
                               float* pre16);
int asw_split_weights_f16(const float* w, size_t n, uint16_t* hi, uint16_t* lo, int32_t* w_shift);
int asw_f16x3_overflow_count(int reset, uint32_t* count);
int asw_convgemm_stats_tiles(int M_out, int N);
#define ASW_RESIDUE_MAX_TAPS 8
#define ASW_RESIDUE_MAX_SHIFT 2
typedef struct asw_residue_stage {
  int32_t residue;
  int32_t chunk;
  int32_t rows;
  int32_t first_row;
  int32_t ntaps;
  int32_t tap[ASW_RESIDUE_MAX_TAPS];
  int32_t shift[ASW_RESIDUE_MAX_TAPS];
  int32_t kstep[ASW_RESIDUE_MAX_TAPS];
} asw_residue_stage;
int asw_residue_schedule(int taps, int stride, int dil, int pad, int Cin, int BK, int BM, int m0, int has_skip,
                         asw_residue_stage* out, int cap, int* n_stages, int* max_shift);

int asw_gn_glu(const float* raw, const float* stats, int n_partials, const float* gamma,
               const float* beta, int B, int T, int C, float eps, float* out, void* stream);
int asw_gn_finalize(const float* stats, int n_partials, int B, int T, int C, float eps, float* mr, void* stream);

int asw_attention(const float* qkv, int B, int L, int d, int nhead, float* ctx, void* stream);
int asw_attention_prec(const float* qkv, int B, int L, int d, int nhead, int precision, float* ctx, void* stream);

int asw_overlap_add_unnorm(const float* D, int B, int F, int ldd, int taps, int hop,
                           int t, int trim_left, int trim_right, float bias, const float* mean,
                           const float* std, float* out, void* stream);
int asw_overlap_add_parts(const float* D, int nparts, int B, int F, int ldd, int taps, int hop,
                          int t, int trim_left, int trim_right, float bias, const float* mean,
                          const float* std, float* out, void* stream);

int asw_energies(const float* y, int B, int T, int window, double* scratch, double* out,
                 void* stream);

int asw_add_layernorm(const float* x, const float* resid, const float* gamma, const float* beta,
                      int rows, int N, float eps, float* out, void* stream);

int asw_center_rows(float* y, int B, int T, void* stream);

int asw_pair_sisdr(const float* y, int n, int T, double* out, void* stream);

int asw_segment_sisdr(const float* y, int n, int T, const int32_t* segments, const int32_t* seg_count,
                      int kmax, double* out, void* stream);

size_t asw_voiced_segments_workspace_bytes(int n, int T);
int asw_voiced_segments(const float* y, int n, int T, double thr, double Q, int32_t* segments, int kcap,
                        int32_t* counts, double* ms, void* workspace, size_t workspace_bytes, void* stream);

size_t asw_fine_clusters_workspace_bytes(const int32_t* bounds_host, int G);
int asw_fine_clusters(const float* y, int N, int T, const int32_t* bounds_host, int G, const double* energies,
                      const double* gate, const double* group_gate, double min_trigger, double ratio, void* workspace,
                      size_t workspace_bytes, int32_t* order, int32_t* label, double* gram, void* stream);

size_t asw_global_clusters_workspace_bytes(int n);
int asw_global_clusters(const double* full, const double* seg, const int32_t* counts, const uint8_t* near, int n, int K,
                        double sim_db, double win_hi, double win_lo, double best_hi, double best_lo, void* workspace,
                        size_t workspace_bytes, int32_t* label, uint8_t* merge_or_null, void* stream);

size_t asw_coarse_select_workspace_bytes(int N, int cap);
int asw_coarse_select(const double* energies, const double* dis1, const int32_t* best_or_null, int N, double thr1,
                      int relative, double rel, int cap, void* workspace, size_t workspace_bytes, int32_t* kept,
                      int32_t* counts, double* thr, void* stream);

size_t asw_bss_eval_sdr_workspace_bytes(const int32_t* counts_host, int K, int R, int T, int flen);
int asw_bss_eval_sdr(const float* ref, const float* est, const int32_t* counts_host, int K, int R, int T, int flen,
                     double* sdr, int32_t* status, void* workspace, size_t workspace_bytes, void* stream);

size_t asw_bss_eval_sources_workspace_bytes(const int32_t* counts_host, int K, int R, int T, int flen, int all_pairs);
int asw_bss_eval_sources(const float* ref, const float* est, const int32_t* counts_host, int K, int R, int T, int flen,
                         int all_pairs, double* sdr, double* sir, double* sar, int32_t* status, void* workspace,
                         size_t workspace_bytes, void* stream);

size_t asw_cross_sisdr_workspace_bytes(const int32_t* est_counts_host, const int32_t* ref_counts_host, int K, int T);
int asw_cross_sisdr(const float* est, const float* ref, const int32_t* est_counts_host, const int32_t* ref_counts_host,
                    int K, int T, double* out, int32_t* status, void* workspace, size_t workspace_bytes, void* stream);

int asw_search_area(const double* points, int n_pts, const double* mic, int M, double* offset,
                    double* width, const double* ub, double sound_speed, double fs, int* n_children,
                    double** child_offset, double** child_width, int** child_count, int** child_index);
void asw_free(void* p);

int asw_cube_select(const double* offsets, int ny, int nx, int nz, int P, int y0, int y1, int x0, int x1,
                    const double* lo, const double* hi, int32_t* out_idx, int64_t cap, int64_t* count);
int asw_cube_select_planes(const double* planes, int ny, int nx, int nz, int P, int y0, int y1, int x0, int x1,
                    const double* lo, const double* hi, int32_t* out_idx, int64_t cap, int64_t* count);

int asw_srp_frames(int window, int nfft, int hop);
int asw_srp_cross_spectra(const float* mix, int M, int T, int window, int step, int n_windows,
                          int nfft, int hop, int nbins, int nb_pad, float tol,
                          const float* twiddle, const int32_t* pair_i, const int32_t* pair_j,
                          int P, float* xf_scratch, float* cc, void* stream);
int asw_srp_map(const float* cc, int n_windows, int nbins, int P, const double* tau, int G, int M,
                const double* omega, const int32_t* pair_i, const int32_t* pair_j,
                float* part_scratch, float* out, void* stream);

int asw_pruner_covariance(const float* mix, int M, int T, int window, int step, int n_windows,
                          int nfft, int hop, int bin0, int nbins, double* cov, double* magsum,
                          void* stream);
int asw_hermitian_eigh(const double* a, int n, int M, double* evals, double* evecs, void* stream);
int asw_music_map(const double* evecs, int n_windows, int nbins, int M, const double* tau, int G,
                  const double* omega, double* p_scratch, double* max_scratch, float* out,
                  void* stream);
int asw_tops_map(const double* evecs, const double* magsum, int n_windows, int nbins, int bin0,
                 int M, const double* delta, int G, double coef, double* q_scratch,
                 int32_t* max_bin, float* out, void* stream);

int asw_geom_lookup_planes(const double* ys, int ny, const double* xs, int nx, const double* zs, int nz,
                           const double* mics, int M, double C, double FS, double* planes, void* stream);
int asw_geom_voxel_map(const double* xs, int Lx, const double* ys, int Ly, const double* zs, int Lz,
                       const double* mics, int M, const double* border, const double* centre, double C,
                       double FS, double resolution, int32_t* q, uint8_t* valid, double* dis_matrix,
                       void* stream);
int asw_geom_label(const int32_t* q, const uint8_t* valid, int Lx, int Ly, int Lz, int P,
                   uint32_t* adj_scratch, int32_t* flag_scratch, int32_t* labels, int* sweeps, void* stream);
int64_t asw_geom_workspace_bytes(int n_voxels);
int asw_geom_compact(const int32_t* labels, const int32_t* q, const double* xs, int Lx, const double* ys, int Ly,
                     const double* zs, int Lz, const double* mics, int M, const double* centre, double C,
                     void* workspace, int64_t workspace_bytes, int32_t* power_index, int32_t* valid_flat,
                     int32_t* valid_cid, int32_t* members, int32_t* bounds, int32_t* offsets, double* centres,
                     double* tau, double* delta, int* counts, void* stream);
int64_t asw_geom_lattice_workspace_bytes(int n_points, int P);
int asw_geom_lattice(const double* planes, int P, int ny, int nx, int nz, const double* xs, const double* ys,
                     const double* zs, const double* border, double width, void* workspace,
                     int64_t workspace_bytes, int32_t* cells, int32_t* bounds, int32_t* members, double* centres,
                     int* counts, void* stream);
int64_t asw_lattice_nms_workspace_bytes(int N, int P);
int asw_lattice_nms(const int32_t* cells, int N, int P, const double* scores, int radius, void* workspace,
                    int64_t workspace_bytes, int32_t* best, int32_t* degree, void* stream);

int asw_frame_blocks(const float* mix, int M, int Ttot, const int32_t* starts, int K, int T, float* out, void* stream);
int asw_stitch_blocks(const float* rows, int N, const double* taper, const int32_t* starts, const int32_t* row_of, int K,
                      int S, int T, int Ttot, float* out, void* stream);

#define ASW_ORACLE_IRM 0
#define ASW_ORACLE_IBM 1
int asw_stft(const float* x, int R, int N, double* z, void* stream);
size_t asw_istft_workspace_bytes(int R, int F);
int asw_istft(const double* z, int R, int F, int N, double* out, void* workspace, size_t workspace_bytes, void* stream);
size_t asw_oracle_masks_workspace_bytes(const int32_t* counts_host, const int32_t* lengths_host, int K);
int asw_oracle_masks(const float* mix, const float* ref, const int32_t* counts_host, const int32_t* lengths_host, int K,
                     int stride, int kind, double alpha, double theta, double* out, void* workspace, size_t workspace_bytes,
                     void* stream);

size_t asw_room_rir_workspace_bytes(int K, int M, int n_src);
int asw_room_rir(const double* rooms_host, const double* absorption_host, const int32_t* max_orders_host, const double* src_host,
                 const double* mics_host, const int32_t* counts_host, int K, int M, double fs, int length, double* rir,
                 void* workspace, size_t workspace_bytes, void* stream);
size_t asw_room_convolve_workspace_bytes(const int32_t* counts_host, int K, int M, int length, int T);
int asw_room_convolve(const float* dry, const double* rir, const int32_t* counts_host, int K, int M, int length, int T,
                      double* premix, double* mix, void* workspace, size_t workspace_bytes, void* stream);

size_t asw_colored_noise_workspace_bytes(int rows, int T, int max_rows_per_pass);
int asw_colored_noise(const int64_t* row_key_host, const int32_t* row_id_host, int rows, int T, double exponent, int max_rows_per_pass,
                      double* out, void* workspace, size_t workspace_bytes, void* stream);
size_t asw_train_batch_workspace_bytes(int items, int S_max, int M);
int asw_train_batch(const float* mix, int K, int M, int T, int items, int S_max, const int32_t* item_mix_host, const int32_t* shifts_host,
                    const int32_t* counts_host, const double* pink_level_host, const double* white_level_host,
                    const int64_t* white_key_host, const double* pink, void* out, int out_f64, void* workspace, size_t workspace_bytes,
                    void* stream);
int asw_train_losses(const float* est, const float* gt, int N, int T, double* out, void* stream);

#ifdef __cplusplus
}
#endif
#endif
```

Before: 2521 candidates/s.

## Carry layer-0 halo rows across consecutive tiles in fused resstack pair kernel

Adds a carried-halo variant of the two-layer fused residual stack kernel. Each block walks a run of contiguous tiles and keeps the layer-0 output halo rows in registers, so the next tile does not recompute them. Later tiles also skip the halo overlap when staging and reuse the layer parameter table already in LDS. The cost is fewer blocks in the grid (runs instead of tiles) and serial work within each block, which may reduce parallelism for small batches.

Result: faster. 2554 candidates/s, median of 6 (+1.3%).

```diff
diff --git a/acousticswarms-speech_amd/csrc/asw_common.cpp b/acousticswarms-speech_amd/csrc/asw_common.cpp
--- a/acousticswarms-speech_amd/csrc/asw_common.cpp
+++ b/acousticswarms-speech_amd/csrc/asw_common.cpp
@@ -135,6 +135,7 @@
 std::mutex g_mu;
 bool g_on = false;
 bool g_detail = false;
+bool g_form = true;
 std::vector<Rec> g_recs;
 std::vector<hipEvent_t> g_pool;
 hipEvent_t take_event() {
@@ -151,6 +152,7 @@
   return b;
 }
 bool prof_detail() { return g_detail; }
+bool prof_form() { return g_form; }
 ProfScope::ProfScope(hipStream_t s, const std::string& name, double work, double bytes) : slot(-1), stream(s) {
   if (!g_on) return;
   std::lock_guard<std::mutex> lk(g_mu);
@@ -171,7 +173,8 @@
   for (auto& r : asw::g_recs) { asw::g_pool.push_back(r.e0); asw::g_pool.push_back(r.e1); }
   asw::g_recs.clear();
   asw::g_on = on != 0;
-  asw::g_detail = on == 2;
+  asw::g_detail = on == 2 || on == 3;
+  asw::g_form = on != 2;
   return ASW_OK;
 }
 
diff --git a/acousticswarms-speech_amd/csrc/asw_common.h b/acousticswarms-speech_amd/csrc/asw_common.h
--- a/acousticswarms-speech_amd/csrc/asw_common.h
+++ b/acousticswarms-speech_amd/csrc/asw_common.h
@@ -84,6 +84,7 @@
 namespace asw {
 std::string prof_name(const char* base, int bm, int bn, int bk, bool ln, bool stats);
 bool prof_detail();
+bool prof_form();
 struct ProfScope {
   ProfScope(hipStream_t s, const std::string& name, double work, double bytes = 0.0);
   ~ProfScope();
diff --git a/acousticswarms-speech_amd/csrc/resstack.hip b/acousticswarms-speech_amd/csrc/resstack.hip
--- a/acousticswarms-speech_amd/csrc/resstack.hip
+++ b/acousticswarms-speech_amd/csrc/resstack.hip
@@ -1,3 +1,5 @@
+#include <algorithm>
+#include <cstdlib>
 #include <type_traits>
 
 #include "asw_common.h"
@@ -38,6 +40,7 @@
   const half8* Pre_l;
   float pre_up, pre_down;
   int B, T, taps, ntile, BM, img_rows;
+  int nrun, run_q, run_long0;
   float eps;
   LayerDev L[MAXL];
 };
@@ -92,11 +95,13 @@
   return __builtin_bit_cast(half8, __builtin_amdgcn_raw_buffer_load_b128(r, row >= 0 ? row * 16 : (int)0x80000000, 0, 0));
 }
 
-template <bool POLY, int PH>
+template <bool POLY, int PH, bool CARRY = false>
 struct RowMap {
   static constexpr int BMJ = R0 / PH;
   static_assert(BMJ % 32 == 0, "a row fragment must stay inside one phase");
   int T, taps, dil0, pad0, jb, pb, m0, BM, n_img, halo0;
+  int shift;
+  int glu_lo, glu_hi;
 
   __device__ __forceinline__ RowMap(int tile, const KArgs& p) : T(p.T), taps(p.taps), dil0(p.L[0].dil), pad0(p.L[0].pad) {
     const int n_pb = POLY ? (dil0 + PH - 1) / PH : 1;
@@ -107,13 +112,25 @@
     n_img = POLY ? PH * rj() : R0 + 2 * pad0;
     halo0 = p.L[0].halo;
   }
+  __device__ __forceinline__ RowMap(int s, int j, bool last, const KArgs& p) : T(p.T), taps(p.taps), dil0(p.L[0].dil), pad0(p.L[0].pad) {
+    static_assert(CARRY && !POLY, "carried halo: contiguous tiles");
+    const bool head = j == 0;
+    jb = pb = 0;
+    halo0 = p.L[0].halo;
+    m0 = head ? s : s + p.BM + (j - 1) * R0;
+    BM = head ? p.BM : R0;
+    n_img = R0 + 2 * pad0;
+    shift = head ? 0 : 2 * halo0;
+    glu_lo = head ? m0 : m0 + halo0;
+    glu_hi = last ? m0 + BM : m0 + BM + halo0;
+  }
   __device__ __forceinline__ int rj() const { return BMJ + taps - 1; }
 
   __device__ __forceinline__ ImgSrc staged_from(int irow) const {
     int g;
     bool ok = irow < n_img;
     if (!POLY) {
-      g = m0 - halo0 - pad0 + irow;
+      g = m0 - halo0 - pad0 + (CARRY ? shift : 0) + irow;
     } else {
       const int ph = pb * PH + irow / rj();
       const int jj = jb * BMJ + irow % rj() - (taps - 1) / 2;
@@ -122,14 +139,14 @@
     }
     return {g, ok && g >= 0 && g < T};
   }
-  __device__ __forceinline__ bool delivers(int g) const { return g >= m0 && g < m0 + BM; }
+  __device__ __forceinline__ bool delivers(int g) const { return CARRY ? g >= glu_lo && g < glu_hi : g >= m0 && g < m0 + BM; }
 
   __device__ __forceinline__ int image_row(int frow) const { return POLY ? (frow / BMJ) * rj() + frow % BMJ : frow; }
   __device__ __forceinline__ int tap_rows(const LayerDev& Ld) const { return POLY ? 1 : Ld.dil; }
   __device__ __forceinline__ int centre_rows(const LayerDev& Ld, bool first) const { return POLY ? (taps - 1) / 2 : first ? pad0 : Ld.pad; }
 
   __device__ __forceinline__ bool handed_on(int frow, int halo) const {
-    const int t = m0 - halo + frow;
+    const int t = m0 - halo + (CARRY ? shift : 0) + frow;
     return t >= 0 && t < T;
   }
   __device__ __forceinline__ int phase(int frow) const { return pb * PH + frow / BMJ; }
@@ -164,12 +181,20 @@
 }
 __device__ __forceinline__ float4 group4(const floatx16& a, int q) { return make_float4(a[q * 4 + 0], a[q * 4 + 1], a[q * 4 + 2], a[q * 4 + 3]); }
 
-template <int NL>
-__device__ __forceinline__ void load_layer_vectors(const KArgs& p, float* tab, int tid) {
+template <int STRIDE>
+struct Tab {
+  static_assert(STRIDE % 16 == 0, "float4 groups");
+  float* p;
+  __device__ __forceinline__ float4& at(int word) const { return *reinterpret_cast<float4*>(p + word * (STRIDE / 16)); }
+  __device__ __forceinline__ Tab layer(int li) const { return {p + li * 192 * (STRIDE / 16)}; }
+};
+
+template <int NL, typename TabT>
+__device__ __forceinline__ void load_layer_vectors(const KArgs& p, TabT tab, int tid) {
   for (int i = tid; i < NL * 3 * 16; i += NTHR) {
     const int li = i / 48, w = (i - li * 48) / 16, c4 = i & 15;
     const float* src = w == 0 ? p.L[li].bias : w == 1 ? p.L[li].gamma : p.L[li].beta;
-    reinterpret_cast<float4*>(tab)[i] = *reinterpret_cast<const float4*>(src + c4 * 4);
+    tab.at(i * 4) = *reinterpret_cast<const float4*>(src + c4 * 4);
   }
 }
 
@@ -226,8 +251,9 @@
   }
 }
 
-template <int NL, typename Map>
-__device__ __forceinline__ void source_layer0(const KArgs& p, const Map& map, int b, float* tab, int tid, floatx16 (&acc)[TM][2]) {
+template <int NL, bool WOFS, typename Map, typename TabT>
+__device__ __forceinline__ void source_layer0(const KArgs& p, const Map& map, int b, TabT tab, bool load_tab, int wofs, int tid,
+                                              floatx16 (&acc)[TM][2]) {
   const LayerDev& Ld = p.L[0];
   const int T = map.T, lane = tid & 63, wid = tid >> 6, h = lane >> 5;
   const __amdgpu_buffer_rsrc_t rH = src_rsrc(p.src_h + (long)b * T, T), rL = src_rsrc(p.src_l + (long)b * T, T);
@@ -250,13 +276,13 @@
     constexpr int kg = decltype(kgc)::value;
 #pragma unroll
     for (int cb = 0; cb < 2; ++cb) {
-      if constexpr (kg < 4) frag_load<3>(Ld.Wh, Ld.Wl, (long)kg * 2 + cb, lane, wh[slot][cb], wl[slot][cb]);
-      else frag_load<3>(p.Pre_h, p.Pre_l, (long)cb, lane, wh[slot][cb], wl[slot][cb]);
+      if constexpr (kg < 4) frag_load<3>(Ld.Wh, Ld.Wl, (long)kg * 2 + cb + (WOFS ? wofs : 0), lane, wh[slot][cb], wl[slot][cb]);
+      else frag_load<3>(p.Pre_h, p.Pre_l, (long)cb + (WOFS ? wofs : 0), lane, wh[slot][cb], wl[slot][cb]);
     }
   };
   wload(std::integral_constant<int, 0>{}, 0);
   wload(std::integral_constant<int, 1>{}, 1);
-  load_layer_vectors<NL>(p, tab, tid);
+  if (load_tab) load_layer_vectors<NL>(p, tab, tid);
   __syncthreads();
   auto kstep = [&](auto ksc) {
     constexpr int ks = decltype(ksc)::value;
@@ -274,7 +300,7 @@
 #pragma unroll
   for (int i = 0; i < TM; ++i) {
     for_each_group(h, [&](int cb, int q, int c0) __attribute__((always_inline)) {
-      const float4 bi = *reinterpret_cast<const float4*>(tab + c0);
+      const float4 bi = tab.at(c0);
       const float bv[4] = {bi.x, bi.y, bi.z, bi.w};
 #pragma unroll
       for (int j = 0; j < 4; ++j)
@@ -285,9 +311,9 @@
   }
 }
 
-template <int NTERM, typename Map>
-__device__ __forceinline__ void conv_layer(const KArgs& p, const LayerDev& Ld, const Map& map, const char* img, int nf, int lane,
-                                           int wid, floatx16 (&acc)[TM][2]) {
+template <int NTERM, bool WOFS, typename Map>
+__device__ __forceinline__ void conv_layer(const KArgs& p, const LayerDev& Ld, const Map& map, const char* img, int nf, int wofs,
+                                           int lane, int wid, floatx16 (&acc)[TM][2]) {
   const int taps = map.taps, h = lane >> 5;
   const int tapstep = map.tap_rows(Ld) * RS;
   auto run = [&](auto nfc) {
@@ -300,9 +326,14 @@
       a[i][0] = acc[i][0];
       a[i][1] = acc[i][1];
     }
-    kloop<NF, 2, QD, NTERM>(
-        a, taps, [&](int tap, int i) __attribute__((always_inline)) { return img + xb[i] + tap * tapstep; }, Ld.Wh, Ld.Wl,
-        [](int kg, int cb) __attribute__((always_inline)) { return (long)kg * 2 + cb; }, lane);
+    if constexpr (WOFS)
+      kloop<NF, 2, QD, NTERM>(
+          a, taps, [&](int tap, int i) __attribute__((always_inline)) { return img + xb[i] + tap * tapstep; }, Ld.Wh, Ld.Wl,
+          [wofs](int kg, int cb) __attribute__((always_inline)) { return (long)kg * 2 + cb + wofs; }, lane);
+    else
+      kloop<NF, 2, QD, NTERM>(
+          a, taps, [&](int tap, int i) __attribute__((always_inline)) { return img + xb[i] + tap * tapstep; }, Ld.Wh, Ld.Wl,
+          [](int kg, int cb) __attribute__((always_inline)) { return (long)kg * 2 + cb; }, lane);
 #pragma unroll
     for (int i = 0; i < NF; ++i) { acc[i][0] = a[i][0]; acc[i][1] = a[i][1]; }
   };
@@ -310,8 +341,8 @@
   else if (nf == 1) run(std::integral_constant<int, 1>{});
 }
 
-template <bool IN_ACC, bool FUSED_VAR, typename Map>
-__device__ __forceinline__ void finish_rows(const KArgs& p, const LayerDev& Ld, const Map& map, const char* img, const float* tb,
+template <bool IN_ACC, bool FUSED_VAR, typename Map, typename TabT>
+__device__ __forceinline__ void finish_rows(const KArgs& p, const LayerDev& Ld, const Map& map, const char* img, const TabT tb,
                                             bool first, int nf, int lane, int wid, floatx16 (&acc)[TM][2]) {
   const int h = lane >> 5;
   const int cpad = map.centre_rows(Ld, first);
@@ -319,7 +350,7 @@
     const char* rrow = img + (map.image_row(frag_row(wid, i, lane)) + cpad) * RS;
     float s = 0.f;
     for_each_group(h, [&](int cb, int q, int c0) __attribute__((always_inline)) {
-      const float4 bi = *reinterpret_cast<const float4*>(tb + c0);
+      const float4 bi = tb.at(c0);
       const half4 rh = *reinterpret_cast<const half4*>(rrow + IMG_HI + c0 * 2);
       const half4 rl = *reinterpret_cast<const half4*>(rrow + IMG_LO + c0 * 2);
       const float bv[4] = {bi.x, bi.y, bi.z, bi.w};
@@ -354,8 +385,8 @@
     d += __shfl_xor(d, 32, 64);
     const float rstd = 1.0f / sqrtf(d * (1.0f / C) + p.eps);
     for_each_group(h, [&](int cb, int q, int c0) __attribute__((always_inline)) {
-      const float4 g4 = *reinterpret_cast<const float4*>(tb + 64 + c0);
-      const float4 b4 = *reinterpret_cast<const float4*>(tb + 128 + c0);
+      const float4 g4 = tb.at(64 + c0);
+      const float4 b4 = tb.at(128 + c0);
       const float gv[4] = {g4.x, g4.y, g4.z, g4.w}, be[4] = {b4.x, b4.y, b4.z, b4.w};
 #pragma unroll
       for (int j = 0; j < 4; ++j) acc[i][cb][q * 4 + j] = (acc[i][cb][q * 4 + j] - mean) * rstd * gv[j] + be[j];
@@ -364,12 +395,12 @@
 }
 
 template <int NTERM, typename Map>
-__device__ __forceinline__ void hand_over(const LayerDev& Ld, const Map& map, char* img, int nf, int lane, int wid,
+__device__ __forceinline__ void hand_over(const LayerDev& Ld, const Map& map, char* img, int row0, int nf, int lane, int wid,
                                           const floatx16 (&acc)[TM][2]) {
   for_each_fragment(nf, [&](int i) __attribute__((always_inline)) {
     const int frow = frag_row(wid, i, lane);
     const bool inside = map.handed_on(frow, Ld.halo);
-    char* wrow = img + frow * RS;
+    char* wrow = img + (row0 + frow) * RS;
     for_each_group(lane >> 5, [&](int cb, int q, int c0) __attribute__((always_inline)) {
       float4 v = group4(acc[i][cb], q);
       if (!inside) v = make_float4(0.f, 0.f, 0.f, 0.f);
@@ -502,7 +533,7 @@
 
   extern __shared__ __align__(16) char smem[];
   char* img = smem;
-  float* tab = reinterpret_cast<float*>(smem + (size_t)p.img_rows * RS);
+  const Tab<16> tab = {reinterpret_cast<float*>(smem + (size_t)p.img_rows * RS)};
 
   const int tid = threadIdx.x, lane = tid & 63, wid = tid >> 6;
   int idx;
@@ -531,13 +562,13 @@
       for (int cb = 0; cb < 2; ++cb)
 #pragma unroll
         for (int r = 0; r < 16; ++r) acc[i][cb][r] = 0.f;
-    if constexpr (fed) source_layer0<NL>(p, map, b, tab, tid, acc);
-    else conv_layer<NTERM>(p, Ld, map, img, nf, lane, wid, acc);
+    if constexpr (fed) source_layer0<NL, false>(p, map, b, tab, true, 0, tid, acc);
+    else conv_layer<NTERM, false>(p, Ld, map, img, nf, 0, lane, wid, acc);
     clk.mark_after(2 + 2 * li, acc[0][0][0]);
-    finish_rows<fed, UP>(p, Ld, map, img, tab + li * 192, li == 0, nf, lane, wid, acc);
+    finish_rows<fed, UP>(p, Ld, map, img, tab.layer(li), li == 0, nf, lane, wid, acc);
     if constexpr (li < NL - 1) {
       if constexpr (!fed) __syncthreads();
-      hand_over<NTERM>(Ld, map, img, nf, lane, wid, acc);
+      hand_over<NTERM>(Ld, map, img, 0, nf, lane, wid, acc);
       __syncthreads();
     } else if constexpr (UP) {
       up_feed<NTERM>(p, p.u, Ld, map, b, tile, smem, tid, acc);
@@ -552,6 +583,92 @@
   clk.report<NL>();
 }
 
+constexpr int CQ = 3;
+template <bool GLU, int NTERM, bool SRC>
+__global__ __launch_bounds__(NTHR) __attribute__((amdgpu_waves_per_eu(2)))
+void resstack64_carry_kernel(const KArgs p) {
+  static_assert(!SRC || (!GLU && NTERM == 3), "source-fed layer 0: f16x3");
+  constexpr int NL = 2;
+  using Map = RowMap<false, 1, true>;
+
+  extern __shared__ __align__(16) char smem[];
+  char* img = smem;
+  const Tab<RS> tab = {reinterpret_cast<float*>(smem + IMG_LO + C * 2)};
+
+  const int tid = threadIdx.x, lane = tid & 63, wid = tid >> 6;
+  int idx;
+  if (!xcd_tile_run(p.B * p.nrun, idx)) return;
+  const int b = idx / p.nrun, run = idx - b * p.nrun;
+  const int s = run * (p.BM + (p.run_q - 1) * R0) + max(run - p.run_long0, 0) * R0;
+  const int n = p.run_q + (run >= p.run_long0 ? 1 : 0);
+  const int crows = 2 * p.L[0].halo;
+
+  PhaseClock clk;
+  floatx16 acc[TM][2];
+  half8 carry[CQ];
+#pragma unroll 1
+  for (int j = 0; j < n; ++j) {
+    const bool steady = j > 0;
+    const Map map(s, j, j == n - 1, p);
+    if (map.m0 >= p.T) break;
+    int wofs = 0;
+    asm volatile("" : "+v"(wofs));
+    wofs = __builtin_amdgcn_readfirstlane(wofs);
+
+    clk.mark(0);
+    if constexpr (!SRC) {
+      if (steady) __syncthreads();
+      else load_layer_vectors<NL>(p, tab, tid);
+      stage_rows<GLU, NTERM>(p, map, b, img, tid);
+      __syncthreads();
+    }
+    clk.mark(1);
+
+    auto layer = [&](auto lic) __attribute__((always_inline)) {
+      constexpr int li = decltype(lic)::value;
+      constexpr bool fed = SRC && li == 0;
+      const LayerDev& Ld = p.L[li];
+      const int nf = (li == 0 || steady ? NW * TM : Ld.nfrag) - wid * TM;
+#pragma unroll
+      for (int i = 0; i < TM; ++i)
+#pragma unroll
+        for (int cb = 0; cb < 2; ++cb)
+#pragma unroll
+          for (int r = 0; r < 16; ++r) acc[i][cb][r] = 0.f;
+      if constexpr (fed) source_layer0<NL, true>(p, map, b, tab, !steady, wofs, tid, acc);
+      else conv_layer<NTERM, true>(p, Ld, map, img, nf, wofs, lane, wid, acc);
+      clk.mark_after(2 + 2 * li, acc[0][0][0]);
+      finish_rows<fed, false>(p, Ld, map, img, tab.layer(li), li == 0, nf, lane, wid, acc);
+      if constexpr (li == 0) {
+        if constexpr (!fed) __syncthreads();
+        hand_over<NTERM>(Ld, map, img, steady ? crows : 0, nf, lane, wid, acc);
+        if (steady) {
+#pragma unroll
+          for (int k = 0; k < CQ; ++k) {
+            const int c = tid + k * NTHR;
+            if (c < crows * 16) *reinterpret_cast<half8*>(img + (c >> 4) * RS + (c & 15) * 16) = carry[k];
+          }
+        }
+        __syncthreads();
+      } else {
+        store_rows(p, map, b, nf, lane, wid, acc);
+      }
+      clk.mark(3 + 2 * li);
+    };
+    layer(std::integral_constant<int, 0>{});
+    layer(std::integral_constant<int, 1>{});
+    clk.report<NL>();
+
+    if (j + 1 < n) {
+#pragma unroll
+      for (int k = 0; k < CQ; ++k) {
+        const int c = tid + k * NTHR;
+        if (c < crows * 16) carry[k] = *reinterpret_cast<const half8*>(img + (map.BM + (c >> 4)) * RS + (c & 15) * 16);
+      }
+    }
+  }
+}
+
 template <bool GLU, bool SRC, bool UP>
 double stack_bytes(const KArgs& k) {
   const double rows = (double)k.B * k.T;
@@ -560,20 +677,35 @@
   return rows * C * 4 * (GLU ? 3 : 2);
 }
 
-template <int NL, int PH, bool POLY, bool GLU, bool SRC, bool UP>
+template <int NL, int PH, bool POLY, bool GLU, int NTERM, bool SRC, bool UP, bool CARRY>
+constexpr auto stack_kernel() {
+  if constexpr (CARRY) {
+    static_assert(NL == 2 && !POLY && !UP, "carried halo: the fused pair on contiguous tiles, not UpFeed");
+    return &resstack64_carry_kernel<GLU, NTERM, SRC>;
+  } else {
+    return &resstack64_kernel<NL, PH, POLY, GLU, NTERM, SRC, UP>;
+  }
+}
+
+template <int NL, int PH, bool POLY, bool GLU, bool SRC, bool UP, bool CARRY = false>
 int launch_stack(const KArgs& k, const UpArgs* up, int precision, size_t smem, double flops, hipStream_t s) {
   char nm[128], detail[48] = "";
-  snprintf(nm, sizeof nm, "resstack64<%d,%dx%d%s%s%s%s>", NL, NW, TM, POLY ? (PH == 1 ? ",poly1" : PH == 2 ? ",poly2" : ",poly4") : "",
-           GLU ? ",glu" : "", SRC ? ",src" : "", UP ? ",up" : "");
-  if (asw::prof_detail()) snprintf(detail, sizeof detail, "[B%d M%d d%d]", k.B, k.T, k.L[0].dil);
+  snprintf(nm, sizeof nm, "resstack64<%d,%dx%d%s%s%s%s%s>", NL, NW, TM, POLY ? (PH == 1 ? ",poly1" : PH == 2 ? ",poly2" : ",poly4") : "",
+           CARRY && asw::prof_form() ? ",carry" : "", GLU ? ",glu" : "", SRC ? ",src" : "", UP ? ",up" : "");
+  if (asw::prof_detail()) {
+    if (CARRY && asw::prof_form()) snprintf(detail, sizeof detail, "[B%d M%d d%d r%d]", k.B, k.T, k.L[0].dil, k.nrun);
+    else snprintf(detail, sizeof detail, "[B%d M%d d%d]", k.B, k.T, k.L[0].dil);
+  }
   std::conditional_t<UP, KArgsUp, KArgs> ka;
   static_cast<KArgs&>(ka) = k;
   if constexpr (UP) {
     ka.u = *up;
     flops += 2.0 * k.B * (double)k.T * C * UPN;
   }
-  return asw::launch_pair<resstack64_kernel<NL, PH, POLY, GLU, (SRC || UP) ? 3 : 1, SRC, UP>, resstack64_kernel<NL, PH, POLY, GLU, 3, SRC, UP>>(
-      precision, dim3(xcd_grid_run(k.B * k.ntile)), dim3(NTHR), smem, 160 * 1024, nm, detail, flops, stack_bytes<GLU, SRC, UP>(k), s, ka);
+  return asw::launch_pair<stack_kernel<NL, PH, POLY, GLU, (SRC || UP) ? 3 : 1, SRC, UP, CARRY>(),
+                          stack_kernel<NL, PH, POLY, GLU, 3, SRC, UP, CARRY>()>(
+      precision, dim3(xcd_grid_run(k.B * (CARRY ? k.nrun : k.ntile))), dim3(NTHR), smem, 160 * 1024, nm, detail, flops,
+      stack_bytes<GLU, SRC, UP>(k), s, ka);
 }
 
 template <int NL, int PH, bool POLY>
@@ -595,6 +727,29 @@
   }
   const int BM = R0 - 2 * halo0;
   return {false, 1, BM, BM > 0 ? asw::cdiv(T, BM) : 0};
+}
+
+struct RunPlan { int nrun, q, long0; };
+RunPlan plan_runs(int T, int BM, int want) {
+  const int nrun = std::max(1, std::min(want, asw::cdiv(T, BM)));
+  const int ntile = nrun + asw::cdiv(std::max(T - nrun * BM, 0), R0);
+  return {nrun, ntile / nrun, nrun - ntile % nrun};
+}
+int auto_runs(int T, int BM, int B, int n_cu) {
+  return std::max(1, std::min(asw::cdiv(4 * n_cu, B), T / (BM + R0)));
+}
+int device_cus() {
+  static int cus[64] = {};
+  int dev = 0;
+  if (hipGetDevice(&dev) != hipSuccess || dev < 0 || dev >= 64) return 256;
+  if (!cus[dev] && hipDeviceGetAttribute(&cus[dev], hipDeviceAttributeMultiprocessorCount, dev) != hipSuccess) cus[dev] = 256;
+  return cus[dev];
+}
+bool carry_applies(int T, int n_layers, int BM, int pad0, int halo0, bool up, int runs_per_item) {
+  static const bool off = getenv("ASW_RESSTACK_NO_CARRY") != nullptr;
+  const int rows = R0 + 2 * std::max(pad0, halo0);
+  return !off && runs_per_item >= 0 && n_layers == 2 && !up && T > BM && halo0 > 0 && 2 * halo0 * 16 <= CQ * NTHR &&
+         (size_t)rows * RS <= 80 * 1024 && rows >= 2 * 3 * 16;
 }
 
 int dispatch(const asw_resstack_args& a, KArgs& k, const UpArgs* up, bool glu, double flops, hipStream_t s) {
@@ -622,6 +777,15 @@
     const int r = 32 * k.L[i].nfrag + 2 * k.L[i].pad;
     rows = r > rows ? r : rows;
   }
+  if (carry_applies(a.T, a.n_layers, k.BM, k.L[0].pad, k.L[0].halo, up != nullptr, a.runs_per_item)) {
+    const RunPlan rp = plan_runs(a.T, k.BM, a.runs_per_item > 0 ? a.runs_per_item : auto_runs(a.T, k.BM, a.B, device_cus()));
+    k.nrun = rp.nrun; k.run_q = rp.q; k.run_long0 = rp.long0;
+    k.img_rows = R0 + 2 * std::max(k.L[0].pad, k.L[0].halo);
+    const size_t lds = (size_t)k.img_rows * RS;
+    if (k.src_h) return launch_stack<2, 1, false, false, true, false, true>(k, nullptr, a.precision, lds, flops, s);
+    return glu ? launch_stack<2, 1, false, true, false, false, true>(k, nullptr, a.precision, lds, flops, s)
+               : launch_stack<2, 1, false, false, false, false, true>(k, nullptr, a.precision, lds, flops, s);
+  }
   k.img_rows = rows;
   const size_t smem = (size_t)rows * RS + (size_t)a.n_layers * 3 * 64 * sizeof(float);
   ASW_CHECK_ARG(smem <= 160 * 1024, "resstack: image of %d rows exceeds LDS (dilation %d x %d taps too wide for a contiguous tile)",
@@ -677,6 +841,21 @@
   const TilePlan t = plan_tiles(T, n_layers, dil[0], halo0, glu != 0);
   ASW_CHECK_ARG(t.BM >= R0 / 2, "resstack_tiles: the later layers' halo (%d rows per side) is too wide", halo0);
   return t.ntile;
+}
+
+extern "C" int asw_resstack_runs(int T, int B, int taps, const int32_t* dil, int runs_per_item, int n_cu, int32_t* head_rows,
+                                 int32_t* steady_rows, int32_t* run_start, int32_t* run_tiles, int max_runs) {
+  ASW_CHECK_ARG(T > 0 && B > 0 && taps >= 3 && taps % 2 == 1 && dil && n_cu > 0 && max_runs >= 0, "resstack_runs: bad argument");
+  const int pad0 = dil[0] * (taps - 1) / 2, halo0 = dil[1] * (taps - 1) / 2, BM = R0 - 2 * halo0;
+  if (BM < R0 / 2 || !carry_applies(T, 2, BM, pad0, halo0, false, runs_per_item)) return 0;
+  const RunPlan rp = plan_runs(T, BM, runs_per_item > 0 ? runs_per_item : auto_runs(T, BM, B, n_cu));
+  if (head_rows) *head_rows = BM;
+  if (steady_rows) *steady_rows = R0;
+  for (int r = 0; r < rp.nrun && r < max_runs; ++r) {
+    if (run_start) run_start[r] = r * (BM + (rp.q - 1) * R0) + std::max(r - rp.long0, 0) * R0;
+    if (run_tiles) run_tiles[r] = rp.q + (r >= rp.long0 ? 1 : 0);
+  }
+  return rp.nrun;
 }
 
 extern "C" int asw_resstack64_f16x3(const asw_resstack_args* args, void* stream) {
diff --git a/acousticswarms-speech_amd/native.py b/acousticswarms-speech_amd/native.py
--- a/acousticswarms-speech_amd/native.py
+++ b/acousticswarms-speech_amd/native.py
@@ -140,7 +140,7 @@
                 ("glu_raw", c_void_p), ("glu_mr", c_void_p), ("glu_gamma", c_void_p), ("glu_beta", c_void_p),
                 ("glu_out", c_void_p), ("src_hi", c_void_p), ("src_lo", c_void_p), ("pre_hi", c_void_p), ("pre_lo", c_void_p),
                 ("pre_shift", c_int32), ("up_hi", c_void_p), ("up_lo", c_void_p), ("up_shift", c_int32), ("up_bias", c_void_p),
-                ("up_skip", c_void_p), ("up_out", c_void_p), ("up_stats", c_void_p)]
+                ("up_skip", c_void_p), ("up_out", c_void_p), ("up_stats", c_void_p), ("runs_per_item", c_int32)]
 
 
 RESIDUE_MAX_TAPS = 8
@@ -214,6 +214,8 @@
     "asw_mask_path_f16x3_scaled": (c_int, [POINTER(MaskPathArgs), c_void_p]),
     "asw_resstack64_f16x3": (c_int, [POINTER(ResStackArgs), c_void_p]),
     "asw_resstack_tiles": (c_int, [c_int, c_int, c_int, POINTER(c_int32), c_int]),
+    "asw_resstack_runs": (c_int, [c_int, c_int, c_int, POINTER(c_int32), c_int, c_int, POINTER(c_int32), POINTER(c_int32),
+                                  POINTER(c_int32), POINTER(c_int32), c_int]),
     "asw_up_feed_kperm": (c_int, [c_int]),
     "asw_pack_up_feed_f16": (c_int, [c_void_p, c_int, c_int, c_void_p, c_void_p, POINTER(c_int32)]),
     "asw_compose_source_weights": (c_int, [c_void_p, c_void_p, c_void_p, c_int, c_int, c_void_p, c_void_p]),
diff --git a/acousticswarms-speech_amd/ops.py b/acousticswarms-speech_amd/ops.py
--- a/acousticswarms-speech_amd/ops.py
+++ b/acousticswarms-speech_amd/ops.py
@@ -87,13 +87,14 @@
     torch.cuda.current_stream().synchronize()
 
 
-def resstack(x, layers, taps=7, precision="f16x3", eps=1e-5, glu=None, out=None, glu_out=None):
+def resstack(x, layers, taps=7, precision="f16x3", eps=1e-5, glu=None, out=None, glu_out=None, runs_per_item=0):
     src = x if glu is None else glu[0]
     B, T = src.shape[0], src.shape[1]
     if out is None:
         out = torch.empty((B, T, 64), dtype=torch.float32, device=src.device)
     a, keep = _resstack_args(B, T, layers, taps, precision, eps, x=x, glu=glu, glu_out=glu_out)
     a.out = out.data_ptr()
+    a.runs_per_item = runs_per_item
     _resstack_launch(a)
     return out
 
@@ -116,7 +117,7 @@
     return raw, stats
 
 
-def resstack_src(src_hi, src_lo, pre_w, pre_b, layers, taps=7, eps=1e-5, out=None):
+def resstack_src(src_hi, src_lo, pre_w, pre_b, layers, taps=7, eps=1e-5, out=None, runs_per_item=0):
     import ctypes
     import numpy as np
     B, T = src_hi.shape[0], src_hi.shape[1]
@@ -137,6 +138,7 @@
     a.out = out.data_ptr()
     ph, pl, psh = pack_fragments_f16(torch.from_numpy(pre16).to(dev), 64, 16)
     a.src_hi, a.src_lo, a.pre_hi, a.pre_lo, a.pre_shift = src_hi.data_ptr(), src_lo.data_ptr(), ph.data_ptr(), pl.data_ptr(), psh
+    a.runs_per_item = runs_per_item
     _resstack_launch(a)
     return out
 
diff --git a/include/asw_hip.h b/include/asw_hip.h
--- a/include/asw_hip.h
+++ b/include/asw_hip.h
@@ -245,8 +245,11 @@
   const float* up_skip;
   float* up_out;
   float* up_stats;
+  int32_t runs_per_item;
 } asw_resstack_args;
 int asw_resstack64_f16x3(const asw_resstack_args* args, void* stream);
+int asw_resstack_runs(int T, int B, int taps, const int32_t* dil, int runs_per_item, int n_cu, int32_t* head_rows,
+                      int32_t* steady_rows, int32_t* run_start, int32_t* run_tiles, int max_runs);
 int asw_resstack_tiles(int T, int taps, int n_layers, const int32_t* dil, int glu);
 int asw_up_feed_kperm(int k);
 int asw_pack_up_feed_f16(const float* Wt, int N, int K, uint16_t* hi, uint16_t* lo, int32_t* w_shift);
```
